# kaftanski/fissure-segmentation

Hardware: AMD Instinct MI355X
Metric: points/sec fwd+bwd DGCNN-seg N=2048 k=20 (higher is better)
Workload: dtype f32

## Files before the change

### fissure-segmentation_amd/_lib.py

```python
import ctypes
import os

import torch

_HERE = os.path.dirname(os.path.abspath(__file__))
LIB_PATH = os.environ.get("FSG_HIP_LIB") or os.path.join(_HERE, "libfsg_hip.so")

if not os.path.exists(LIB_PATH):
    raise ImportError(f"{LIB_PATH} not found: build it with `python -c 'import __graft_entry__ as g; g.build()'` "
                      f"or `make -C {os.path.join(_HERE, 'csrc')}`; there is no CPU fallback.")

lib = ctypes.CDLL(LIB_PATH)

_P, _I, _L, _F = ctypes.c_void_p, ctypes.c_int, ctypes.c_int64, ctypes.c_float
SIGNATURES = {
    "fsg_version": ([], _I),
    "fsg_last_error": ([], ctypes.c_char_p),
    "fsg_knn_dense_f32": ([_P, _I, _I, _L, _L, _I, _I, _I, _P, _P, _P, _P], _I),
    "fsg_knn_dense_workspace_bytes": ([_I, _I, _I], ctypes.c_size_t),
    "fsg_knn_dense_ws_f32": ([_P, _I, _I, _L, _L, _I, _I, _I, _P, _P, _P, ctypes.c_size_t, _P], _I),
    "fsg_knn_dense_prepared_f32": ([_P, _I, _I, _I, _I, _I, _P, _P, _P, ctypes.c_size_t, _P], _I),
    "fsg_knn_dense_ws_pq_f32": ([_P, _I, _I, _L, _L, _I, _I, _I, _P, _P, _P, ctypes.c_size_t, _P, _I, _P, _P], _I),
    "fsg_edgeconv_apply_f32": ([_P, _P, _P, _P, _P, _I, _I, _I, _F, _P, _P, _P, ctypes.c_size_t, _P], _I),
    "fsg_edgeconv_apply_pq_f32": ([_P, _P, _P, _P, _P, _I, _I, _I, _F, _P, _P, _P, ctypes.c_size_t, _P, _I, _P, _P], _I),
    "fsg_edge_gather_fwd_f32": ([_P, _P, _P, _I, _I, _I, _I, _P], _I),
    "fsg_edge_gather_bwd_f32": ([_P, _P, _P, _I, _I, _I, _I, _P], _I),
    "fsg_knn_gather_fused_f32": ([_P, _I, _I, _I, _I, _I, _P, _P, _P, _P], _I),
    "fsg_knn_gather_fused_ws_f32": ([_P, _I, _I, _I, _I, _I, _P, _P, _P, ctypes.c_size_t, _P], _I),
    "fsg_edge_gather_fwd_bf16": ([_P, _P, _P, _I, _I, _I, _I, _P], _I),
    "fsg_edge_gather_bwd_bf16": ([_P, _P, _P, _I, _I, _I, _I, _P], _I),
    "fsg_graph_reverse_csr_workspace_bytes": ([_I, _I, _I], ctypes.c_size_t),
    "fsg_graph_reverse_csr": ([_P, _I, _I, _I, _P, _P, _P, _P], _I),
    "fsg_edge_weights_fwd_f32": ([_P, _I, _I, _P, _P], _I),
    "fsg_edge_weights_bwd_f32": ([_P, _I, _I, _P, _P], _I),
    "fsg_edge_weights_many_f32": ([_P, _I, _P], _I),
    "fsg_edgeconv1_workspace_bytes": ([_I, _I, _I], ctypes.c_size_t),
    "fsg_edgeconv1_fwd_f32": ([_P, _P, _P, _P, _P, _P, _I, _I, _I, _I, _I, _F, _F, _F, _P, _P, _P, _P, _P, _P, _P, _P, _P],
                              _I),
    "fsg_edgeconv1_bwd_f32": ([_P, _P, _L, _P, _L, _P, _P, _P, _P, _P, _P, _P, _P, _P, _P, _I, _I, _I, _I, _I, _F, _P, _P,
                               _P, _P, _P, _P], _I),
    "fsg_edgeconv2_workspace_bytes": ([_I, _I, _I, _I], ctypes.c_size_t),
    "fsg_edgeconv2_bwd_workspace_bytes": ([_I, _I, _I, _I], ctypes.c_size_t),
    "fsg_edgeconv2_fwd_f32": ([_P] * 11 + [_I] * 5 + [_F] * 5 + [_P] * 12, _I),
    "fsg_edgeconv2_bwd_f32": ([_P, _P, _L, _P, _L] + [_P] * 16 + [_I] * 5 + [_F] + [_P] * 8, _I),
    "fsg_edgeconv2_fwd_bf16": ([_P] * 11 + [_I] * 5 + [_F] * 5 + [_P] * 12, _I),
    "fsg_edgeconv2_bwd_bf16": ([_P, _P, _L, _P, _L] + [_P] * 16 + [_I] * 5 + [_F] + [_P] * 8, _I),
    "fsg_bn_act_workspace_bytes": ([ctypes.c_long, _I], ctypes.c_size_t),
    "fsg_bn_act_fwd_f32": ([_P, _P, _P, _P, _P, ctypes.c_long, _I, _I, _F, _F, _F, _P, _P, _P, _P, _P], _I),
    "fsg_bn_act_bwd_f32": ([_P, _P, _P, _P, _P, _P, ctypes.c_long, _I, _I, _F, _P, _P, _P, _P, _P], _I),
    "fsg_bn_act_max_workspace_bytes": ([_I, _I, _I], ctypes.c_size_t),
    "fsg_bn_act_max_fwd_f32": ([_P, _P, _P, _P, _P, _I, _I, _I, _I, _F, _F, _F, _P, _P, _P, _P, _P, _P, _P], _I),
    "fsg_bn_act_max_bwd_f32": ([_P, _P, _P, _P, _P, _P, _P, _P, _I, _I, _I, _I, _F, _P, _P, _P, _P], _I),
    "fsg_bn_act_maxavg_workspace_bytes": ([_I, _I, _I], ctypes.c_size_t),
    "fsg_bn_act_maxavg_fwd_f32": ([_P, _P, _P, _P, _P, _I, _I, _I, _I, _F, _F, _F, _P, _P, _P, _P, _P, _P], _I),
    "fsg_bn_act_maxavg_bwd_f32": ([_P, _P, _P, _P, _P, _P, _P, _I, _I, _I, _I, _F, _P, _P, _P, _P, _P], _I),
    "fsg_chamfer_nn_f32": ([_P, _P, _I, _I, _I, _P, _P, _P], _I),
    "fsg_chamfer_nn_bwd_workspace_bytes": ([_I, _I, _I], ctypes.c_size_t),
    "fsg_chamfer_nn_bwd_f32": ([_P, _P, _P, _P, _I, _I, _I, _P, _P, _P, _P], _I),
    "fsg_point_mesh_dist_f32": ([_P, _P, _P, _I, _I, _I, _I, _I, _P, _P, _P, _P], _I),
    "fsg_mesh_labelmap_dist_f32": ([_P, _P, _P, _I, _I, _I, _I, _I, _F, _F, _F, _F, _P, _P, _P, _P], _I),
    "fsg_mesh_labelmap_cover_f32": ([_P, _P, _P, _I, _I, _I, _I, _I, _F, _F, _F, _P, _P], _I),
    "fsg_ensemble_accumulate_workspace_bytes": ([_I, _L], ctypes.c_size_t),
    "fsg_ensemble_accumulate_f32": ([_P, _I, _I, _I, _I, _P, _L, _P, _P, _P], _I),
    "fsg_sample_transform_f32": ([_P, _I, _I, _L, _P, _I, _P, _P, _P], _I),
    "fsg_ssm_decode_bwd_workspace_bytes": ([_I, _I, _I], ctypes.c_size_t),
    "fsg_ssm_decode_fwd_f32": ([_P, _P, _P, _P, _P, _P, _I, _I, _I, _P, _P], _I),
    "fsg_ssm_decode_bwd_f32": ([_P, _P, _P, _P, _P, _P, _I, _I, _I, _P, _P, _P, _P, _P, ctypes.c_size_t, _P], _I),
    "fsg_colsum_narrow_f32": ([_P, _L, _I, _P, _P], _I),
    "fsg_fold_layer1_f32": ([_P, _I, _P, _L, _P, _I, _I, _I, _I, _P, _P], _I),
    "fsg_adam_flat_f32": ([_P, _P, _P, _P, _P, _L, _F, _P, _F, _F, _F, _F, _P], _I),
    "fsg_nnu_loss_workspace_bytes": ([_I], ctypes.c_size_t),
    "fsg_nnu_loss_f32": ([_P, _L, _L, _L, _P, _P, _I, _I, _I, _F, _F, _F, _P, _P, _L, _L, _L, _P, _P], _I),
    "fsg_bn_rows_workspace_bytes": ([ctypes.c_long, _I], ctypes.c_size_t),
    "fsg_bn_rows_fwd_f32": ([_P, _P, _P, _P, _P, _P, ctypes.c_long, _I, _I, _F, _F, _I, _P, _P, _P, _P, _P], _I),
    "fsg_bn_rows_bwd_f32": ([_P, _P, _P, _P, _P, _P, ctypes.c_long, _I, _I, _I, _P, _P, _P, _P, _P, _P], _I),
    "fsg_gemm_small_workspace_bytes": ([_I, _I, _I], ctypes.c_size_t),
    "fsg_gemm_small_f32": ([_P, _L, _L, _P, _L, _L, _P, _P, _L, _I, _I, _I, _P, _P], _I),
    "fsg_gemm_small_rowsum_f32": ([_P, _L, _L, _P, _L, _L, _P, _P, _L, _I, _I, _I, _P, _P, _P], _I),
    "fsg_gemm_small_deferred_f32": ([_P, _L, _L, _P, _L, _L, _P, _L, _I, _I, _I, _P, _P, _P, _P], _I),
    "fsg_gemm_small_reduce_many_f32": ([_P, _P], _I),
    "fsg_gemm_small_bf16": ([_P, _L, _L, _P, _L, _L, _P, _P, _L, _I, _I, _I, _P, _P, _P, _P], _I),
    "fsg_pt_attn_workspace_bytes": ([_I, _I, _I], ctypes.c_size_t),
    "fsg_pt_attn_fwd_f32": ([_P, _P, _P, _P, _P, _L, _P, _I, _I, _I, _I, _P, _P, _P, _P, _P, _P], _I),
    "fsg_pt_attn_bwd_f32": ([_P, _P, _P, _P, _P, _L, _P, _I, _I, _I, _I, _P, _P, _P, _P, _P, _P, _P, _L, _P, _P, _P, _P], _I),
    "fsg_knn_segment_f32": ([_P, _P, _P, _P, _I, _I, _I, _I, _P, _P, _P], _I),
    "fsg_fps_f32": ([_P, _P, _P, _I, _I, _P, _P, _P], _I),
    "fsg_group_gather_fwd_f32": ([_P, _P, _P, _I, _I, _I, _I, _P], _I),
    "fsg_group_gather_bwd_f32": ([_P, _P, _P, _I, _I, _I, _I, _P], _I),
    "fsg_group_xyz_feat_fwd_f32": ([_P, _P, _P, _P, _P, _I, _I, _I, _I, _P], _I),
    "fsg_group_xyz_feat_bwd_f32": ([_P, _P, _P, _I, _I, _I, _I, _P], _I),
    "fsg_rows_max_fwd_f32": ([_P, _P, _P, _I, _I, _I, _P], _I),
    "fsg_rows_max_bwd_f32": ([_P, _P, _P, _I, _I, _I, _P], _I),
    "fsg_interp_fwd_f32": ([_P, _P, _P, _P, _I, _I, _I, _I, _P], _I),
    "fsg_interp_bwd_f32": ([_P, _P, _P, _P, _I, _I, _I, _I, _P], _I),
    "fsg_vec_attn_fwd_f32": ([_P, _P, _P, _P, _P, _I, _I, _I, _I, _P], _I),
    "fsg_vec_attn_bwd_f32": ([_P, _P, _P, _P, _P, _P, _P, _P, _I, _I, _I, _I, _P], _I),
    "fsg_pw_weight_image_bytes": ([_I, _I], ctypes.c_size_t),
    "fsg_pw_weight_image_f32": ([_P, _L, _L, _I, _I, _F, _I, _I, _P, _P], _I),
    "fsg_pw_weight_images_f32": ([_P, _P], _I),
    "fsg_pw_linear_f32": ([_P, _L, _P, _P, _P, _L, _I, _I, _I, _I, _P], _I),
    "fsg_pw_weight_image_bf16": ([_P, _L, _L, _I, _I, _P, _P], _I),
    "fsg_pw_linear_bf16": ([_P, _L, _P, _P, _P, _L, _I, _I, _I, _I, _P], _I),
    "fsg_pw_tn_bf16": ([_P, _I, _P, ctypes.c_size_t, _P, _L, _P], _I),
    "fsg_pw_tile_rows": ([_I], _I),
    "fsg_pw_rowgemm_f32": ([_P, _I, _I, _I, _P], _I),
    "fsg_pw_tn_workspace_bytes": ([_I, _I, _I, _I], ctypes.c_size_t),
    "fsg_pw_tn_f32": ([_P, _I, _P, ctypes.c_size_t, _P, _L, _P, _L, _P], _I),
    "fsg_pw_tn_reduce_f32": ([_P, _P], _I),
    "fsg_pw_bn_finalize_f32": ([_P, _I, _I, _I, _I, _P, _I, _I, _P, _P, _F, _F, _P, _P, _P, _P, _P, _P, _P, _P, _P, _P, _L, _I, _P, _P], _I),
    "fsg_pw_cloud_linear_f32": ([_P, _P, _L, _I, _I, _I, _P, _P], _I),
    "fsg_pw_max_finish_f32": ([_P, _P, _P, _P, _P, _I, _I, _I, _F, _P, _P, _P, _P], _I),
    "fsg_pw_bn_finalize_max_f32": ([_P, _I, _I, _I, _I, _I, _I, _P, _P, _F, _F, _P, _P, _P, _P, _P, _P, _P, _P, _P, _I, _F, _P, _P, _P,
                                   _P], _I),
    "fsg_pw_bnbwd_finalize_f32": ([_P, _I, _I, _I, _L, _I, _P, _P, _P, _I, _P, _P, _P, _P, _P, _P, _P], _I),
    "fsg_pw_logits_bwd_f32": ([_P, _I, _P, _P, _P, _P, _P, _P, _L, _I, _F, _P, _P, _P], _I),
    "fsg_pw_gf_prep_f32": ([_P, _P, _L, _I, _P, _P, _L, _P, _P, _P, _P, _P, _P, _I, _I, _L, _I, _F, _P, _P, _P, _P, _P, _P, _L, _I, _P, _L,
                            _P], _I),
    "fsg_pw_scatter_rows_workspace_bytes": ([_I, _I], ctypes.c_size_t),
    "fsg_pw_scatter_rows_f32": ([_P, _P, _P, _L, _I, _I, _I, _I, _P, _L, _P, _P], _I),
    "fsg_pw_gf_dw_f32": ([_P, _P, _P, _L, _P, _P, _L, _P, _P, _P, _I, _I, _I, _I, _P, _L, _P], _I),
    "fsg_pw_logits_bwd_bias_f32": ([_P, _I, _P, _P, _P, _P, _P, _P, _L, _I, _F, _P, _P, _P, _P], _I),
    "fsg_pw_gf_prep_sort_f32": ([_P, _P, _L, _I, _P, _P, _L, _P, _P, _P, _P, _P, _I, _I, _L, _I, _F, _P, _P, _P, _P, _P, _P, _L, _I, _P,
                                 _L, _P, _I, _P, _P, _P], _I),
    "fsg_pw_tn_reduce_image_f32": ([_P, _I, _I, _I, _I, _F, _I, _I, _P, _P, _L, _P], _I),
    "fsg_pw_rowgemm_scatter_f32": ([_P, _P, _P, _P, _P, _L, _I, _P], _I),
    "fsg_foerstner_dist_f32": ([_P, _I, _I, _I, _I, _P, _I, _P, _P], _I),
    "fsg_nms_keypoints": ([_P, _P, _I, _I, _I, _I, _I, _F, _P, _P, _P], _I),
    "fsg_mind_stats_workspace_bytes": ([_I, _I, _I, _I], ctypes.c_size_t),
    "fsg_mind_stats_f32": ([_P, _I, _I, _I, _I, _I, _I, _I, _P, _P, _I, _P, _P, _P], _I),
    "fsg_mind_eval_f32": ([_P, _I, _I, _I, _I, _I, _I, _I, _P, _P, _P, _I, _P, _P, _P], _I),
    "fsg_mind_eval_kp_f32": ([_P, _I, _I, _I, _I, _I, _I, _P, _P, _P, _I, _P, _P, _I, _P, _P], _I),
    "fsg_fissure_enhance_f32": ([_P, _P, _I, _I, _I, _I, _P, _P, _I, _F, _F, _P, _P, _P, _P], _I),
    "fsg_smooth_threshold_f32": ([_P, _I, _I, _I, _I, _P, _I, _P, _I, _P, _I, _F, _P, _P, _P], _I),
    "fsg_cpd_estep_workspace_bytes": ([_I, _I, _I], ctypes.c_size_t),
    "fsg_cpd_estep_f32": ([_P, _L, _P, _P, _F, _I, _I, _I, _P, _P, _P, _P, _P, ctypes.c_size_t, _P], _I),
    "fsg_random_walk_workspace_bytes": ([_I, _I, _I, _I, _I], ctypes.c_size_t),
    "fsg_random_walk_prep": ([_P, _I, _P, _I, _P, _I, _I, _I, _I, _I, _P, ctypes.c_size_t, _P, _P, _P], _I),
    "fsg_random_walk_iterate": ([_P, _I, _I, _I, _I, _I, _I, _I, _I, _F, _P, ctypes.c_size_t, _P, _P, _P], _I),
    "fsg_random_walk_finish": ([_I, _I, _I, _I, _I, _P, ctypes.c_size_t, _P, _P, _P], _I),
    "fsg_lobes_to_fissures_u8": ([_P, _I, _I, _I, _I, _I, _P, _P], _I),
    "fsg_bits_pack_u8": ([_P, _I, _I, _I, _I, _I, _P, _P], _I),
    "fsg_bits_unpack_u8": ([_P, _I, _I, _I, _I, _P, _P], _I),
    "fsg_bits_window": ([_P, _I, _I, _I, _I, _I, _I, _I, _I, _I, _I, _P, _P], _I),
    "fsg_ball_dilate_bits": ([_P, _I, _I, _I, _I, _I, _I, _I, _I, _I, _I, _P, _P], _I),
    "fsg_cc_workspace_bytes": ([_I, _I, _I, _I], ctypes.c_size_t),
    "fsg_cc_label_bits": ([_P, _I, _I, _I, _I, _I, _P, _P, _P, ctypes.c_size_t, _P], _I),
    "fsg_component_stats_i32": ([_P, _I, _I, _I, _I, _I, _P, _P], _I),
    "fsg_relabel_lut_i32": ([_P, _I, _L, _P, _I, _P, _I, _P], _I),
    "fsg_mesh_reg_workspace_bytes": ([_I, _I], ctypes.c_size_t),
    "fsg_mesh_reg_f32": ([_P, _L, _P, _I, _I, _P, _P, _P, _P, _P, _P, _P, _P, _P, ctypes.c_size_t, _P], _I),
    "fsg_mesh_sample_workspace_bytes": ([_I, _I], ctypes.c_size_t),
    "fsg_mesh_sample_f32": ([_P, _P, _P, _I, _I, _P, _I, _P, _P, _P, _P, ctypes.c_size_t, _P], _I),
    "fsg_mesh_sample_bwd_f32": ([_P, _P, _P, _P, _P, _I, _I, _I, _P, _P], _I),
    "fsg_grid_corners_f32": ([_P, _I, _I, _I, _I, _I, _I, _P, _P, _P], _I),
    "fsg_grid_splat_workspace_bytes": ([_I, _I, _I], ctypes.c_size_t),
    "fsg_grid_splat_sorted_f32": ([_P, _P, _P, _P, _I, _I, _I, _I, _I, _I, _P, _P, ctypes.c_size_t, _P], _I),
    "fsg_grid_sample_f32": ([_P, _P, _P, _I, _I, _I, _I, _I, _I, _I, _P, _P, _P], _I),
    "fsg_psr_spectral_f32": ([_P, _I, _I, _I, _I, ctypes.c_double, _I, _P, _P], _I),
    "fsg_mc_workspace_bytes": ([_I, _I, _I, _I], ctypes.c_size_t),
    "fsg_mc_count_f32": ([_P, _P, _L, _I, _I, _I, _I, _F, _I, _P, ctypes.c_size_t, _P, _P], _I),
    "fsg_mc_count_labels_i32": ([_P, _P, _L, _I, _I, _I, _I, _I, _P, ctypes.c_size_t, _P, _P], _I),
    "fsg_mc_emit_f32": ([_P, _I, _I, _I, _I, _F, _I, _F, _F, _F, _P, ctypes.c_size_t, _P, _L, _L, _P, _P, _P, _P], _I),
    "fsg_mc_emit_labels_i32": ([_P, _I, _I, _I, _I, _I, _I, _F, _F, _F, _P, ctypes.c_size_t, _P, _L, _L, _P, _P, _P, _P], _I),
    "fsg_pcl_normals_f32": ([_P, _P, _P, _I, _I, _I, _I, _P, _P, _P, _P], _I),
    "fsg_orient_normals_workspace_bytes": ([_I, _I], ctypes.c_size_t),
    "fsg_orient_normals_f32": ([_P, _P, _P, _P, _I, _I, _I, _P, ctypes.c_size_t, _P, _P, _P, _P], _I),
    "fsg_face_union_i32": ([_P, _P, _I, _P, _P, _P], _I),
    "fsg_cluster_stats_f64": ([_P, _P, _P, _P, _P, _I, _I, _I, _P, _P, _P, _P], _I),
    "fsg_mesh_keep_flags_u8": ([_P, _I, _P, _I, _P, _P, _P, _I, _I, _I, _F, _F, _F, _P, _P], _I),
    "fsg_mesh_face_flags_u8": ([_P, _I, _I, _P, _P, _P, _P, _P], _I),
    "fsg_mesh_compact_f32": ([_P, _P, _P, _I, _I, _P, _I, _P, _P, _P, _P, _P, _P, _P, _P], _I),
}
for _name, (_args, _res) in SIGNATURES.items():
    _fn = getattr(lib, _name)
    _fn.argtypes, _fn.restype = _args, _res

GRID_TORCH, GRID_SAP = 0, 1
MORPH_MAX_RADIUS = 8
PCL_NORMALS_MAX_K = 64
ORIENT_MAX_POINTS = 1 << 20
RW_BINARY, RW_INTENSITY, RW_MAX_LABELS = 0, 1, 8
KNN_FIX_DIAG, KNN_DROP_FIRST, KNN_FORCE_ROWS, KNN_FORCE_MFMA, KNN_MAX_K = 1, 2, 4, 8, 64
KNN_DBG_HALF_CHUNKS, KNN_DBG_TWO_PHASE, KNN_DBG_ALL_SLOW, KNN_DBG_STATS = 1 << 11, 1 << 21, 1 << 22, 1 << 25
KNN_DBG_STAMPS, KNN_DBG_ONE_LAUNCH, KNN_DBG_BF16 = 1 << 28, 1 << 29, 1 << 30


_timing = None


def start_timing():
    global _timing
    _timing = {}


def stop_timing():
    global _timing
    rec, _timing = _timing, None
    torch.cuda.synchronize()
    return {name: [s.elapsed_time(e) for s, e in evs] for name, evs in (rec or {}).items()}


class PTLayerParams(ctypes.Structure):
    _fields_ = [(n, _P) for n in ("lp1_w", "lp1_b", "bnp_g", "bnp_b", "bnp_rm", "bnp_rv", "lp2_w", "lp2_b", "bn1_g", "bn1_b",
                                  "bn1_rm", "bn1_rv", "lw1_w", "lw1_b", "bn2_g", "bn2_b", "bn2_rm", "bn2_rv", "lw2_w",
                                  "lw2_b")] + [(n, _F) for n in ("eps_p", "eps_1", "eps_2", "mom_p", "mom_1", "mom_2")]


GEMM_REDUCE_MAX_JOBS = 48


class GemmReduceJobs(ctypes.Structure):
    _fields_ = [("part", _P * GEMM_REDUCE_MAX_JOBS), ("C", _P * GEMM_REDUCE_MAX_JOBS), ("rowsum", _P * GEMM_REDUCE_MAX_JOBS),
                ("ldc", _L * GEMM_REDUCE_MAX_JOBS), ("S", _I * GEMM_REDUCE_MAX_JOBS), ("I", _I * GEMM_REDUCE_MAX_JOBS),
                ("J", _I * GEMM_REDUCE_MAX_JOBS), ("blocks", _I * GEMM_REDUCE_MAX_JOBS), ("n", _I)]


class EdgeWeightJobs(ctypes.Structure):
    _fields_ = [("src", _P * 8), ("dst", _P * 8), ("Co", _I * 8), ("C", _I * 8), ("n", _I)]


class PWRowGemmArgs(ctypes.Structure):
    _fields_ = [("A1", _P), ("Y1", _P), ("A2", _P), ("lda1", _L), ("lda2", _L), ("K1", _I), ("K2", _I), ("Bimg", _P),
                ("M", _I), ("N", _I), ("rows_per_cloud", _I), ("alpha", _P), ("delta", _P), ("P", _P), ("Q", _P),
                ("tstride", _I), ("slope", _F), ("C", _P), ("ldc", _L), ("store_n0", _I), ("bias", _P), ("rec", _P),
                ("sgn", _P), ("sel_val", _P), ("sel_arg", _P), ("sel_n", _I), ("Yp", _P), ("ldyp", _L), ("ealpha", _P),
                ("edelta", _P), ("emu", _P), ("er", _P), ("etstride", _I), ("rec2", _P)]


PW_MAX_IMAGE_JOBS = 10


class PWImageJobs(ctypes.Structure):
    _fields_ = [("W", _P * PW_MAX_IMAGE_JOBS), ("stride_n", _L * PW_MAX_IMAGE_JOBS), ("stride_k", _L * PW_MAX_IMAGE_JOBS),
                ("N", _I * PW_MAX_IMAGE_JOBS), ("K", _I * PW_MAX_IMAGE_JOBS), ("ks0", _I * PW_MAX_IMAGE_JOBS),
                ("KS", _I * PW_MAX_IMAGE_JOBS), ("scale", _F * PW_MAX_IMAGE_JOBS), ("image", _P * PW_MAX_IMAGE_JOBS), ("n", _I)]


PW_MAX_REDUCE_JOBS = 6


class PWTnReduceJobs(ctypes.Structure):
    _fields_ = [("workspace", _P * PW_MAX_REDUCE_JOBS), ("C1", _P * PW_MAX_REDUCE_JOBS), ("C2", _P * PW_MAX_REDUCE_JOBS),
                ("ldc1", _L * PW_MAX_REDUCE_JOBS), ("ldc2", _L * PW_MAX_REDUCE_JOBS), ("S", _I * PW_MAX_REDUCE_JOBS),
                ("N1", _I * PW_MAX_REDUCE_JOBS), ("N2", _I * PW_MAX_REDUCE_JOBS), ("N1a", _I * PW_MAX_REDUCE_JOBS), ("n", _I)]


class PWTnArgs(ctypes.Structure):
    _fields_ = [("L1", _P), ("LY1", _P), ("L2", _P), ("ldl1", _L), ("ldl2", _L), ("N1a", _I), ("N1b", _I), ("lpro", _I),
                ("lalpha", _P), ("ldelta", _P), ("lP", _P), ("lQ", _P), ("lts", _I), ("R", _P), ("ldr", _L), ("N2", _I),
                ("rpro", _I), ("ralpha", _P), ("rdelta", _P), ("rts", _I), ("slope", _F), ("M", _I), ("rows_per_cloud", _I),
                ("rows_per_slice", _I), ("ones", _I)]


class PTLayerGrads(ctypes.Structure):
    _fields_ = [(n, _P) for n in ("lp1_w", "lp1_b", "bnp_g", "bnp_b", "lp2_w", "lp2_b", "bn1_g", "bn1_b", "lw1_w", "lw1_b",
                                  "bn2_g", "bn2_b", "lw2_w", "lw2_b")]


_experiments = None


def experiments():
    global _experiments
    if _experiments is None:
        path = os.path.join(_HERE, "libfsg_hip_experiments.so")
        if not os.path.exists(path):
            raise ImportError(f"{path} not found: `make -C {os.path.join(_HERE, 'csrc')} all` builds it")
        x = ctypes.CDLL(path)
        x.fsg_knn_experiment_f32.argtypes, x.fsg_knn_experiment_f32.restype = SIGNATURES["fsg_knn_dense_f32"][0], _I
        x.fsg_last_error.restype = ctypes.c_char_p
        _experiments = x
    return _experiments


def workspace(entry, *dims, device):
    nbytes = getattr(lib, entry + "_workspace_bytes")(*dims)
    return torch.empty(nbytes, dtype=torch.uint8, device=device) if nbytes else None


def call(name, *args):
    if _timing is None:
        rc = getattr(lib, name)(*args)
    else:
        s, e = torch.cuda.Event(enable_timing=True), torch.cuda.Event(enable_timing=True)
        s.record()
        rc = getattr(lib, name)(*args)
        e.record()
        _timing.setdefault(name, []).append((s, e))
    if rc != 0:
        raise RuntimeError(f"{name} failed (code {rc}): {lib.fsg_last_error().decode()}")
```

### fissure-segmentation_amd/csrc/adam.hip

```cpp
#include "fsg_common.h"

namespace {

struct AdamState {
    float step;
    unsigned int ticket;
};

__device__ __forceinline__ void adam_one(float &p, float g, float &m, float &v, float b1, float b2, float eps, float wd,
                                         float step_size, float bc2_sqrt) {
    if (wd != 0.f) g = fmaf(wd, p, g);
    m = m + (1.f - b1) * (g - m);
    v = b2 * v + (1.f - b2) * g * g;
    const float denom = sqrtf(v) / bc2_sqrt + eps;
    p -= step_size * (m / denom);
}

__global__ __launch_bounds__(256) void adam_flat_kernel(float *__restrict__ param, const float *__restrict__ grad,
                                                        float *__restrict__ exp_avg, float *__restrict__ exp_avg_sq,
                                                        AdamState *__restrict__ state, long n, float lr_host,
                                                        const float *__restrict__ lr_dev, float b1, float b2, float eps,
                                                        float wd) {
    __shared__ float sc[2];
    if (threadIdx.x == 0) {
        const double t = (double)state->step + 1.0;
        const double lr = lr_dev ? (double)lr_dev[0] : (double)lr_host;
        sc[0] = (float)(lr / (1.0 - pow((double)b1, t)));
        sc[1] = (float)sqrt(1.0 - pow((double)b2, t));
    }
    __syncthreads();
    const float step_size = sc[0], bc2_sqrt = sc[1];
    const long n4 = n >> 2;
    for (long i = (long)blockIdx.x * 256 + threadIdx.x; i < n4; i += (long)gridDim.x * 256) {
        float4 p = reinterpret_cast<float4 *>(param)[i];
        const float4 g = reinterpret_cast<const float4 *>(grad)[i];
        float4 m = reinterpret_cast<float4 *>(exp_avg)[i];
        float4 v = reinterpret_cast<float4 *>(exp_avg_sq)[i];
        adam_one(p.x, g.x, m.x, v.x, b1, b2, eps, wd, step_size, bc2_sqrt);
        adam_one(p.y, g.y, m.y, v.y, b1, b2, eps, wd, step_size, bc2_sqrt);
        adam_one(p.z, g.z, m.z, v.z, b1, b2, eps, wd, step_size, bc2_sqrt);
        adam_one(p.w, g.w, m.w, v.w, b1, b2, eps, wd, step_size, bc2_sqrt);
        reinterpret_cast<float4 *>(param)[i] = p;
        reinterpret_cast<float4 *>(exp_avg)[i] = m;
        reinterpret_cast<float4 *>(exp_avg_sq)[i] = v;
    }
    if (blockIdx.x == 0 && threadIdx.x < (n & 3)) {
        const long i = (n4 << 2) + threadIdx.x;
        float p = param[i], m = exp_avg[i], v = exp_avg_sq[i];
        adam_one(p, grad[i], m, v, b1, b2, eps, wd, step_size, bc2_sqrt);
        param[i] = p;
        exp_avg[i] = m;
        exp_avg_sq[i] = v;
    }
    __syncthreads();
    if (threadIdx.x == 0) {
        const unsigned int done = atomicAdd(&state->ticket, 1u);
        if (done == gridDim.x - 1) {
            state->step += 1.f;
            state->ticket = 0u;
        }
    }
}

}

extern "C" int fsg_adam_flat_f32(float *param, const float *grad, float *exp_avg, float *exp_avg_sq, void *state, int64_t n,
                                 float lr, const float *lr_dev, float beta1, float beta2, float eps, float weight_decay,
                                 fsg_stream_t stream) {
    FSG_REQUIRE(param && grad && exp_avg && exp_avg_sq && state, "fsg_adam_flat_f32: NULL pointer");
    FSG_REQUIRE(n > 0, "fsg_adam_flat_f32: n=%ld", (long)n);
    FSG_REQUIRE((((uintptr_t)param | (uintptr_t)grad | (uintptr_t)exp_avg | (uintptr_t)exp_avg_sq) & 15) == 0,
                "fsg_adam_flat_f32: the four arrays must be 16-byte aligned");
    FSG_REQUIRE(((uintptr_t)state & 7) == 0, "fsg_adam_flat_f32: state must be 8-byte aligned");
    FSG_REQUIRE(beta1 >= 0.f && beta1 < 1.f && beta2 >= 0.f && beta2 < 1.f && eps >= 0.f,
                "fsg_adam_flat_f32: bad hyper-parameters beta1=%g beta2=%g eps=%g", beta1, beta2, eps);
    long blocks = ((n >> 2) + 255) / 256;
    if (blocks < 1) blocks = 1;
    if (blocks > 1024) blocks = 1024;
    hipLaunchKernelGGL(adam_flat_kernel, dim3((unsigned)blocks), dim3(256), 0, (hipStream_t)stream, param, grad, exp_avg,
                       exp_avg_sq, (AdamState *)state, (long)n, lr, lr_dev, beta1, beta2, eps, weight_decay);
    FSG_CHECK_LAUNCH("fsg_adam_flat_f32");
    return FSG_OK;
}
```

### fissure-segmentation_amd/csrc/small_gemm.hip

```cpp

#include "fsg_common.h"

namespace {

constexpr int TI = 64, TJ = 64, TK = 32, LDT = 65;
constexpr int LPT = TI * TK / 256;

__global__ __launch_bounds__(256) void gemm_small_kernel(const float *__restrict__ A, long sai, long sak,
                                                         const float *__restrict__ B, long sbk, long sbj,
                                                         const float *__restrict__ bias, float *__restrict__ C, long ldc,
                                                         int I, int J, int K, int kchunk, float *__restrict__ part,
                                                         float *__restrict__ rowsum) {
    __shared__ float As[TK * LDT], Bs[TK * LDT];
    const int tid = threadIdx.x, wave = __builtin_amdgcn_readfirstlane(tid >> 6), lane = tid & 63, ql = lane & 31, half = lane >> 5;
    const int i0 = blockIdx.x * TI, j0 = blockIdx.y * TJ;
    const int kbeg = blockIdx.z * kchunk, kend = min(K, kbeg + kchunk);
    const int wi = (wave >> 1) * 32, wj = (wave & 1) * 32;
    const bool a_kfast = sak == 1, b_kfast = sbk == 1;
    f32x16 acc;
#pragma unroll
    for (int e = 0; e < 16; ++e) acc[e] = 0.f;
    float av[LPT], bv[LPT];
    auto fetch = [&](int k0) {
#pragma unroll
        for (int r = 0; r < LPT; ++r) {
            const int t = r * 256 + tid;
            const int ai = a_kfast ? t / TK : t % TI, ak = a_kfast ? t % TK : t / TI;
            const int bj = b_kfast ? t / TK : t % TJ, bk = b_kfast ? t % TK : t / TJ;
            av[r] = (i0 + ai < I && k0 + ak < kend) ? A[(long)(i0 + ai) * sai + (long)(k0 + ak) * sak] : 0.f;
            bv[r] = (j0 + bj < J && k0 + bk < kend) ? B[(long)(k0 + bk) * sbk + (long)(j0 + bj) * sbj] : 0.f;
        }
    };
    const bool do_rs = rowsum != nullptr && blockIdx.y == 0 && tid < TI;
    float rs = 0.f;
    if (kbeg < kend) fetch(kbeg);
    for (int k0 = kbeg; k0 < kend; k0 += TK) {
        __syncthreads();
#pragma unroll
        for (int r = 0; r < LPT; ++r) {
            const int t = r * 256 + tid;
            const int ai = a_kfast ? t / TK : t % TI, ak = a_kfast ? t % TK : t / TI;
            const int bj = b_kfast ? t / TK : t % TJ, bk = b_kfast ? t % TK : t / TJ;
            As[ak * LDT + ai] = av[r];
            Bs[bk * LDT + bj] = bv[r];
        }
        __syncthreads();
        if (k0 + TK < kend) fetch(k0 + TK);
        if (do_rs) {
#pragma unroll
            for (int kk = 0; kk < TK; ++kk) rs += As[kk * LDT + tid];
        }
#pragma unroll
        for (int s = 0; s < TK / 2; ++s)
            acc = __builtin_amdgcn_mfma_f32_32x32x2f32(As[(2 * s + half) * LDT + wi + ql], Bs[(2 * s + half) * LDT + wj + ql],
                                                       acc, 0, 0, 0);
    }
    if (do_rs && i0 + tid < I) {
        if (part) part[(long)gridDim.z * I * J + (long)blockIdx.z * I + i0 + tid] = rs;
        else rowsum[i0 + tid] = rs;
    }
    const int col = j0 + wj + ql;
    if (col >= J) return;
    if (part) {
        float *dst = part + (long)blockIdx.z * I * J;
#pragma unroll
        for (int e = 0; e < 16; ++e) {
            const int row = i0 + wi + (e & 3) + 8 * (e >> 2) + 4 * half;
            if (row < I) dst[(long)row * J + col] = acc[e];
        }
    } else {
        const float bb = bias ? bias[col] : 0.f;
#pragma unroll
        for (int e = 0; e < 16; ++e) {
            const int row = i0 + wi + (e & 3) + 8 * (e >> 2) + 4 * half;
            if (row < I) C[(long)row * ldc + col] = acc[e] + bb;
        }
    }
}

typedef unsigned short u16;
constexpr int LDH = TK + 8;
__device__ __forceinline__ u16 to_bf16(float x) {
    const __bf16 h = (__bf16)x;
    return __builtin_bit_cast(u16, h);
}
__global__ __launch_bounds__(256) void gemm_small_bf16_kernel(const float *__restrict__ A, long sai, long sak,
                                                              const float *__restrict__ B, long sbk, long sbj,
                                                              const float *__restrict__ bias, float *__restrict__ C, long ldc,
                                                              int I, int J, int K, int kchunk, float *__restrict__ part,
                                                              float *__restrict__ rowsum) {
    __shared__ __attribute__((aligned(16))) u16 As[TI * LDH], Bs[TJ * LDH];
    const int tid = threadIdx.x, wave = __builtin_amdgcn_readfirstlane(tid >> 6), lane = tid & 63, ql = lane & 31, half = lane >> 5;
    const int i0 = blockIdx.x * TI, j0 = blockIdx.y * TJ;
    const int kbeg = blockIdx.z * kchunk, kend = min(K, kbeg + kchunk);
    const int wi = (wave >> 1) * 32, wj = (wave & 1) * 32;
    const bool a_kfast = sak == 1, b_kfast = sbk == 1;
    f32x16 acc;
#pragma unroll
    for (int e = 0; e < 16; ++e) acc[e] = 0.f;
    float av[LPT], bv[LPT];
    auto fetch = [&](int k0) {
#pragma unroll
        for (int r = 0; r < LPT; ++r) {
            const int t = r * 256 + tid;
            const int ai = a_kfast ? t / TK : t % TI, ak = a_kfast ? t % TK : t / TI;
            const int bj = b_kfast ? t / TK : t % TJ, bk = b_kfast ? t % TK : t / TJ;
            av[r] = (i0 + ai < I && k0 + ak < kend) ? A[(long)(i0 + ai) * sai + (long)(k0 + ak) * sak] : 0.f;
            bv[r] = (j0 + bj < J && k0 + bk < kend) ? B[(long)(k0 + bk) * sbk + (long)(j0 + bj) * sbj] : 0.f;
        }
    };
    const bool do_rs = rowsum != nullptr && blockIdx.y == 0 && tid < TI;
    float rs = 0.f;
    if (kbeg < kend) fetch(kbeg);
    for (int k0 = kbeg; k0 < kend; k0 += TK) {
        __syncthreads();
#pragma unroll
        for (int r = 0; r < LPT; ++r) {
            const int t = r * 256 + tid;
            const int ai = a_kfast ? t / TK : t % TI, ak = a_kfast ? t % TK : t / TI;
            const int bj = b_kfast ? t / TK : t % TJ, bk = b_kfast ? t % TK : t / TJ;
            As[ai * LDH + ak] = to_bf16(av[r]);
            Bs[bj * LDH + bk] = to_bf16(bv[r]);
        }
        __syncthreads();
        if (k0 + TK < kend) fetch(k0 + TK);
        if (do_rs) {
#pragma unroll
            for (int kk = 0; kk < TK; ++kk) rs += __uint_as_float((unsigned)As[tid * LDH + kk] << 16);
        }
#pragma unroll
        for (int s = 0; s < TK / 16; ++s) {
            const bf16x8 a = *reinterpret_cast<const bf16x8 *>(&As[(wi + ql) * LDH + 16 * s + 8 * half]);
            const bf16x8 b = *reinterpret_cast<const bf16x8 *>(&Bs[(wj + ql) * LDH + 16 * s + 8 * half]);
            acc = __builtin_amdgcn_mfma_f32_32x32x16_bf16(a, b, acc, 0, 0, 0);
        }
    }
    if (do_rs && i0 + tid < I) {
        if (part) part[(long)gridDim.z * I * J + (long)blockIdx.z * I + i0 + tid] = rs;
        else rowsum[i0 + tid] = rs;
    }
    const int col = j0 + wj + ql;
    if (col >= J) return;
    if (part) {
        float *dst = part + (long)blockIdx.z * I * J;
#pragma unroll
        for (int e = 0; e < 16; ++e) {
            const int row = i0 + wi + (e & 3) + 8 * (e >> 2) + 4 * half;
            if (row < I) dst[(long)row * J + col] = acc[e];
        }
    } else {
        const float bb = bias ? bias[col] : 0.f;
#pragma unroll
        for (int e = 0; e < 16; ++e) {
            const int row = i0 + wi + (e & 3) + 8 * (e >> 2) + 4 * half;
            if (row < I) C[(long)row * ldc + col] = acc[e] + bb;
        }
    }
}

__global__ __launch_bounds__(256) void gemm_small_reduce_flat_kernel(const float *__restrict__ part, int S, long IJ, int J,
                                                                     const float *__restrict__ bias, float *__restrict__ C,
                                                                     long ldc, int I, float *__restrict__ rowsum) {
    const long t = (long)blockIdx.x * 256 + threadIdx.x;
    if (rowsum && t >= IJ && t < IJ + I) {
        float a = 0.f;
        for (int s = 0; s < S; ++s) a += part[(long)S * IJ + (long)s * I + (t - IJ)];
        rowsum[t - IJ] = a;
    }
    if (t >= IJ) return;
    float a = 0.f;
    for (int s = 0; s < S; ++s) a += part[(long)s * IJ + t];
    const long row = t / J;
    const int col = (int)(t - row * J);
    C[row * ldc + col] = a + (bias ? bias[col] : 0.f);
}

__global__ __launch_bounds__(256) void gemm_small_reduce_kernel(const float *__restrict__ part, int S, long IJ, int J,
                                                                const float *__restrict__ bias, float *__restrict__ C,
                                                                long ldc, int I, float *__restrict__ rowsum) {
    __shared__ float red[16][17];
    const int o = threadIdx.x & 15, sl = threadIdx.x >> 4;
    const long t = (long)blockIdx.x * 16 + o;
    const long nb = (IJ + 15) / 16;
    if (rowsum && (long)blockIdx.x >= nb) {
        const long ri = ((long)blockIdx.x - nb) * 16 + o;
        float a = 0.f;
        if (ri < I)
            for (int s = sl; s < S; s += 16) a += part[(long)S * IJ + (long)s * I + ri];
        red[sl][o] = a;
        __syncthreads();
        if (sl == 0 && ri < I) {
            float r = 0.f;
#pragma unroll
            for (int i = 0; i < 16; ++i) r += red[i][o];
            rowsum[ri] = r;
        }
        return;
    }
    float a = 0.f;
    if (t < IJ)
        for (int s = sl; s < S; s += 16) a += part[(long)s * IJ + t];
    red[sl][o] = a;
    __syncthreads();
    if (sl == 0 && t < IJ) {
        float r = 0.f;
#pragma unroll
        for (int i = 0; i < 16; ++i) r += red[i][o];
        const long row = t / J;
        const int col = (int)(t - row * J);
        C[row * ldc + col] = r + (bias ? bias[col] : 0.f);
    }
}

__global__ __launch_bounds__(256) void gemm_small_reduce_many_kernel(fsg_gemm_reduce_jobs jobs) {
    int j = 0;
    long b = blockIdx.x;
    while (j < jobs.n - 1 && b >= jobs.blocks[j]) { b -= jobs.blocks[j]; ++j; }
    const float *part = jobs.part[j];
    const int S = jobs.S[j], I = jobs.I[j], J = jobs.J[j];
    const long IJ = (long)I * J, t = b * 256 + threadIdx.x;
    float *rowsum = jobs.rowsum[j];
    if (rowsum && t >= IJ && t < IJ + I) {
        float a = 0.f;
        for (int s = 0; s < S; ++s) a += part[(long)S * IJ + (long)s * I + (t - IJ)];
        rowsum[t - IJ] = a;
    }
    if (t >= IJ) return;
    float a = 0.f;
#pragma unroll 8
    for (int s = 0; s < S; ++s) a += part[(long)s * IJ + t];
    const long row = t / J;
    const int col = (int)(t - row * J);
    jobs.C[j][row * jobs.ldc[j] + col] = a;
}

inline int splits_for(int I, int J, int K) {
    constexpr int min_k = 64;
    const long tiles = (long)fsg_cdiv(I, TI) * fsg_cdiv(J, TJ);
    if (tiles >= 256 || K < 2 * min_k) return 1;
    long s = (1024 + tiles - 1) / tiles;
    const long smax = K / min_k;
    if (s > smax) s = smax;
    if (s > 128) s = 128;
    return s < 1 ? 1 : (int)s;
}

}

extern "C" size_t fsg_gemm_small_workspace_bytes(int I, int J, int K) {
    if (I <= 0 || J <= 0 || K <= 0) return 0;
    const int s = splits_for(I, J, K);
    return s > 1 ? sizeof(float) * (size_t)s * ((size_t)I * (size_t)J + (size_t)I) : 0;
}

extern "C" int fsg_gemm_small_rowsum_f32(const float *A, int64_t sa_i, int64_t sa_k, const float *B, int64_t sb_k, int64_t sb_j,
                                         const float *bias, float *C, int64_t ldc, int I, int J, int K, float *rowsum,
                                         void *workspace, fsg_stream_t stream);

extern "C" int fsg_gemm_small_f32(const float *A, int64_t sa_i, int64_t sa_k, const float *B, int64_t sb_k, int64_t sb_j,
                                  const float *bias, float *C, int64_t ldc, int I, int J, int K, void *workspace,
                                  fsg_stream_t stream) {
    return fsg_gemm_small_rowsum_f32(A, sa_i, sa_k, B, sb_k, sb_j, bias, C, ldc, I, J, K, nullptr, workspace, stream);
}

namespace {
int gemm_small_launch(const float *A, int64_t sa_i, int64_t sa_k, const float *B, int64_t sb_k, int64_t sb_j, const float *bias,
                      float *C, int64_t ldc, int I, int J, int K, float *rowsum, void *workspace, int *deferred_splits,
                      fsg_stream_t stream, bool bf16 = false);
}

extern "C" int fsg_gemm_small_rowsum_f32(const float *A, int64_t sa_i, int64_t sa_k, const float *B, int64_t sb_k, int64_t sb_j,
                                         const float *bias, float *C, int64_t ldc, int I, int J, int K, float *rowsum,
                                         void *workspace, fsg_stream_t stream) {
    return gemm_small_launch(A, sa_i, sa_k, B, sb_k, sb_j, bias, C, ldc, I, J, K, rowsum, workspace, nullptr, stream);
}

extern "C" int fsg_gemm_small_deferred_f32(const float *A, int64_t sa_i, int64_t sa_k, const float *B, int64_t sb_k, int64_t sb_j,
                                           float *C, int64_t ldc, int I, int J, int K, float *rowsum, void *workspace, int *splits,
                                           fsg_stream_t stream) {
    FSG_REQUIRE(splits, "fsg_gemm_small_deferred_f32: NULL splits");
    return gemm_small_launch(A, sa_i, sa_k, B, sb_k, sb_j, nullptr, C, ldc, I, J, K, rowsum, workspace, splits, stream);
}

extern "C" int fsg_gemm_small_bf16(const float *A, int64_t sa_i, int64_t sa_k, const float *B, int64_t sb_k, int64_t sb_j,
                                   const float *bias, float *C, int64_t ldc, int I, int J, int K, float *rowsum, void *workspace,
                                   int *splits, fsg_stream_t stream) {
    FSG_REQUIRE(!(splits && bias), "fsg_gemm_small_bf16: a deferred product takes no bias");
    return gemm_small_launch(A, sa_i, sa_k, B, sb_k, sb_j, bias, C, ldc, I, J, K, rowsum, workspace, splits, stream, true);
}

extern "C" int fsg_gemm_small_reduce_many_f32(const fsg_gemm_reduce_jobs *jobs, fsg_stream_t stream) {
    FSG_REQUIRE(jobs && jobs->n >= 1 && jobs->n <= FSG_GEMM_REDUCE_MAX_JOBS, "fsg_gemm_small_reduce_many_f32: bad job count");
    fsg_gemm_reduce_jobs j = *jobs;
    long total = 0;
    for (int i = 0; i < j.n; ++i) {
        FSG_REQUIRE(j.part[i] && j.C[i] && j.S[i] >= 1 && j.I[i] > 0 && j.J[i] > 0 && j.ldc[i] >= j.J[i],
                    "fsg_gemm_small_reduce_many_f32: bad job %d", i);
        j.blocks[i] = (int)fsg_cdiv((long)j.I[i] * j.J[i] + (j.rowsum[i] ? j.I[i] : 0), 256L);
        total += j.blocks[i];
    }
    FSG_REQUIRE(total < (1L << 31), "fsg_gemm_small_reduce_many_f32: too many outputs");
    hipLaunchKernelGGL(gemm_small_reduce_many_kernel, dim3((unsigned)total), dim3(256), 0, (hipStream_t)stream, j);
    FSG_CHECK_LAUNCH("fsg_gemm_small_reduce_many_f32");
    return FSG_OK;
}

namespace {
int gemm_small_launch(const float *A, int64_t sa_i, int64_t sa_k, const float *B, int64_t sb_k, int64_t sb_j, const float *bias,
                      float *C, int64_t ldc, int I, int J, int K, float *rowsum, void *workspace, int *deferred_splits,
                      fsg_stream_t stream, bool bf16) {
    FSG_REQUIRE(A && B && C, "fsg_gemm_small_f32: NULL pointer");
    FSG_REQUIRE(I > 0 && J > 0 && K > 0 && ldc >= J, "fsg_gemm_small_f32: bad shape I=%d J=%d K=%d ldc=%ld", I, J, K, (long)ldc);
    FSG_REQUIRE(fsg_cdiv(J, TJ) <= 65535, "fsg_gemm_small_f32: J too large");
    const int S = splits_for(I, J, K);
    FSG_REQUIRE(S == 1 || workspace, "fsg_gemm_small_f32: this shape needs the workspace");
    hipStream_t st = (hipStream_t)stream;
    int kchunk = fsg_cdiv(fsg_cdiv(K, S), TK) * TK;
    const int S_eff = fsg_cdiv(K, kchunk);
    float *part = S_eff > 1 ? (float *)workspace : nullptr;
    if (bf16)
        hipLaunchKernelGGL(gemm_small_bf16_kernel, dim3(fsg_cdiv(I, TI), fsg_cdiv(J, TJ), S_eff), dim3(256), 0, st, A, (long)sa_i,
                           (long)sa_k, B, (long)sb_k, (long)sb_j, bias, C, (long)ldc, I, J, K, kchunk, part, rowsum);
    else
        hipLaunchKernelGGL(gemm_small_kernel, dim3(fsg_cdiv(I, TI), fsg_cdiv(J, TJ), S_eff), dim3(256), 0, st, A, (long)sa_i,
                           (long)sa_k, B, (long)sb_k, (long)sb_j, bias, C, (long)ldc, I, J, K, kchunk, part, rowsum);
    FSG_CHECK_LAUNCH("fsg_gemm_small_f32");
    if (deferred_splits) {
        *deferred_splits = part ? S_eff : 0;
        return FSG_OK;
    }
    if (part) {
        const long IJ = (long)I * J, outs = IJ + (rowsum ? I : 0);
        if (S_eff >= 16)
            hipLaunchKernelGGL(gemm_small_reduce_kernel, dim3(fsg_cdiv(IJ, 16) + (rowsum ? fsg_cdiv(I, 16) : 0)), dim3(256), 0, st, part,
                               S_eff, IJ, J, bias, C, (long)ldc, I, rowsum);
        else
            hipLaunchKernelGGL(gemm_small_reduce_flat_kernel, dim3(fsg_cdiv(outs, 256)), dim3(256), 0, st, part, S_eff, IJ, J,
                               bias, C, (long)ldc, I, rowsum);
        FSG_CHECK_LAUNCH("fsg_gemm_small_f32/reduce");
    }
    return FSG_OK;
}
}
```

### fissure-segmentation_amd/functional.py

```python
import contextlib as _contextlib
import ctypes
import os as _os

import torch

from . import _lib


def _need_gpu(*tensors):
    for t in tensors:
        if t is not None and not t.is_cuda:
            raise RuntimeError("fissure_segmentation_amd runs on the GPU only (got a CPU tensor); "
                               "the CPU restatement lives in oracle/ and is test infrastructure")


def _p(t):
    return ctypes.c_void_p(t.data_ptr() if t is not None else 0)


def _stream():
    return ctypes.c_void_p(torch.cuda.current_stream().cuda_stream)


def _f32c(t):
    return t.detach().to(torch.float32).contiguous()


def _amp_fwd(fn):
    return torch.amp.custom_fwd(fn, device_type="cuda", cast_inputs=torch.float32)


def _amp_bwd(fn):
    return torch.amp.custom_bwd(fn, device_type="cuda")


def no_autocast():
    if torch.is_autocast_enabled("cuda"):
        return torch.autocast("cuda", enabled=False)
    return _contextlib.nullcontext()


_mfma_mode = "f32"


def set_mfma_operands(kind):
    global _mfma_mode
    if kind not in ("f32", "bf16"):
        raise ValueError("MFMA operand type must be 'f32' or 'bf16'")
    _mfma_mode = kind


@_contextlib.contextmanager
def mfma_operands(kind):
    global _mfma_mode
    old = _mfma_mode
    set_mfma_operands(kind)
    try:
        yield
    finally:
        _mfma_mode = old


def bf16_operands():
    return _mfma_mode == "bf16"


def _ambient_bf16():
    return torch.is_autocast_enabled("cuda") and torch.get_autocast_dtype("cuda") == torch.bfloat16


_deterministic = bool(_os.environ.get("FSG_DETERMINISTIC"))


def set_deterministic(flag=True):
    global _deterministic
    _deterministic = bool(flag)


def deterministic():
    return _deterministic or torch.are_deterministic_algorithms_enabled()


def knn_graph(x, k, c_knn=None, fix_diag=True, drop_first=False, return_dist=False, force_rows_kernel=False,
              _debug_flags=0, out=None, prepared=None, pq_weight=None):
    _need_gpu(x)
    if x.dim() != 3:
        raise ValueError(f"expected (B,C,N), got {tuple(x.shape)}")
    x = x.detach()
    if x.dtype != torch.float32:
        x = x.float()
    if x.stride(2) != 1:
        x = x.contiguous()
    B, C, N = x.shape
    c_knn = C if c_knn is None else c_knn
    if out is not None:
        if out.shape != (B, N, k) or out.dtype != torch.int32 or not out.is_contiguous() or out.device != x.device:
            raise ValueError("knn_graph: `out` must be a contiguous (B,N,k) int32 tensor on the input's device")
        idx = out
    else:
        idx = torch.empty(B, N, k, dtype=torch.int32, device=x.device)
    dist = torch.empty(B, N, k, dtype=torch.float32, device=x.device) if return_dist else None
    flags = (_lib.KNN_FIX_DIAG if fix_diag else 0) | (_lib.KNN_DROP_FIRST if drop_first else 0) | \
        (_lib.KNN_FORCE_ROWS if force_rows_kernel else 0) | _debug_flags
    if prepared is not None and c_knn == C and not return_dist and not force_rows_kernel and not _debug_flags:
        ws, x_pm = prepared
        with torch.cuda.device(x.device):
            _lib.call("fsg_knn_dense_prepared_f32", _p(x_pm), B, N, C, k, flags, _p(idx), None, _p(ws), ws.numel() * ws.element_size(),
                      _stream())
        return idx
    xx = _lib.workspace("fsg_knn_dense", B, N, c_knn, device=x.device)
    ws_bytes = xx.numel() if xx is not None else 0
    if pq_weight is not None:
        rows = pq_weight.shape[0]
        if (C == c_knn and c_knn <= 4 and tuple(pq_weight.shape) == (rows, C) and 256 % rows == 0 and not return_dist and
                not (_debug_flags & _lib.KNN_FORCE_MFMA)):
            pq = torch.empty(B, N, rows, dtype=torch.float32, device=x.device)
            with torch.cuda.device(x.device):
                _lib.call("fsg_knn_dense_ws_pq_f32", _p(x), B, N, x.stride(0), x.stride(1), c_knn, k, flags, _p(idx), None, _p(xx),
                          ws_bytes, _p(_f32c(pq_weight.detach())), rows, _p(pq), _stream())
            return idx, pq
    with torch.cuda.device(x.device):
        rc = 3
        if flags & _lib.KNN_FORCE_MFMA:
            xl = _lib.experiments()
            rc = xl.fsg_knn_experiment_f32(_p(x), B, N, x.stride(0), x.stride(1), c_knn, k, flags, _p(idx), _p(dist), _p(xx),
                                           _stream())
            if rc not in (0, 3):
                raise RuntimeError(xl.fsg_last_error().decode())
        if rc == 3:
            _lib.call("fsg_knn_dense_ws_f32", _p(x), B, N, x.stride(0), x.stride(1), c_knn, k, flags & ~_lib.KNN_FORCE_MFMA, _p(idx),
                      _p(dist), _p(xx), ws_bytes, _stream())
    if pq_weight is not None:
        return idx, None
    return (idx, dist) if return_dist else idx


class _EdgeGather(torch.autograd.Function):
    @staticmethod
    @_amp_fwd
    def forward(ctx, x, idx):
        B, C, N = x.shape
        k = idx.shape[2]
        half = x.dtype == torch.bfloat16
        xc = x.detach().contiguous() if half else _f32c(x)
        out = torch.empty(B, 2 * C, N, k, dtype=xc.dtype, device=x.device)
        with torch.cuda.device(x.device):
            _lib.call("fsg_edge_gather_fwd_bf16" if half else "fsg_edge_gather_fwd_f32", _p(xc), _p(idx), _p(out), B, C, N, k,
                      _stream())
        ctx.save_for_backward(idx)
        ctx.shape = (B, C, N, k)
        ctx.half = half
        return out

    @staticmethod
    @_amp_bwd
    def backward(ctx, g):
        (idx,) = ctx.saved_tensors
        B, C, N, k = ctx.shape
        half = ctx.half and g.dtype == torch.bfloat16
        g = g.detach().contiguous() if half else _f32c(g)
        gx = torch.empty(B, C, N, dtype=torch.float32, device=g.device)
        with torch.cuda.device(g.device):
            _lib.call("fsg_edge_gather_bwd_bf16" if half else "fsg_edge_gather_bwd_f32", _p(g), _p(idx), _p(gx), B, C, N, k,
                      _stream())
        return (gx.to(torch.bfloat16) if ctx.half else gx), None


def knn_edge_features(x, k, knn_only_over_coords=False):
    _need_gpu(x)
    xc = _f32c(x)
    B, C, N = xc.shape
    idx = torch.empty(B, N, k, dtype=torch.int32, device=x.device)
    edge = torch.empty(B, 2 * C, N, k, dtype=torch.float32, device=x.device)
    c_knn = 3 if knn_only_over_coords else C
    ws = _lib.workspace("fsg_knn_dense", B, N, c_knn, device=x.device)
    with torch.cuda.device(x.device):
        _lib.call("fsg_knn_gather_fused_ws_f32", _p(xc), B, C, N, k, c_knn, _p(idx), _p(edge), _p(ws), ws.numel(), _stream())
    return edge, idx


def edge_features(x, idx):
    _need_gpu(x, idx)
    if idx.dtype != torch.int32:
        idx = idx.to(torch.int32)
    return _EdgeGather.apply(x, idx.contiguous())


SMALL_GEMM_FLOPS = 6e8


def gemm_small(a, sa_i, sa_k, b, sb_k, sb_j, bias, I, J, K, rowsum=False, defer=False, bf16=False):
    out = torch.empty(I, J, dtype=torch.float32, device=a.device)
    ws = _lib.workspace("fsg_gemm_small", I, J, K, device=a.device)
    rs = torch.empty(I, dtype=torch.float32, device=a.device) if rowsum else None
    with torch.cuda.device(a.device):
        if defer and bias is None:
            splits = ctypes.c_int(0)
            if bf16:
                _lib.call("fsg_gemm_small_bf16", _p(a), sa_i, sa_k, _p(b), sb_k, sb_j, None, _p(out), J, I, J, K, _p(rs), _p(ws),
                          ctypes.byref(splits), _stream())
            else:
                _lib.call("fsg_gemm_small_deferred_f32", _p(a), sa_i, sa_k, _p(b), sb_k, sb_j, _p(out), J, I, J, K, _p(rs), _p(ws),
                          ctypes.byref(splits), _stream())
            if splits.value > 1:
                _defer_reduce((ws, out.data_ptr(), rs.data_ptr() if rs is not None else None, splits.value, I, J, a.device))
        elif bf16:
            _lib.call("fsg_gemm_small_bf16", _p(a), sa_i, sa_k, _p(b), sb_k, sb_j, _p(bias), _p(out), J, I, J, K, _p(rs), _p(ws), None,
                      _stream())
        else:
            _lib.call("fsg_gemm_small_rowsum_f32", _p(a), sa_i, sa_k, _p(b), sb_k, sb_j, _p(bias), _p(out), J, I, J, K, _p(rs),
                      _p(ws), _stream())
    return (out, rs) if rowsum else out


_pending_reduces = []
_defer_weight_grads = True


def set_deferred_weight_grads(flag):
    global _defer_weight_grads
    _defer_weight_grads = bool(flag)


def _grad_targets(w):
    if w.is_leaf:
        return (w,)
    return getattr(w, "_fsg_grad_unread", None)


def _may_defer(targets):
    return (_defer_weight_grads and targets is not None and not torch.is_grad_enabled() and
            all(p.grad is None for p in targets))


def flush_deferred_reduces():
    global _pending_reduces
    jobs, _pending_reduces = _pending_reduces, []
    for i0 in range(0, len(jobs), _lib.GEMM_REDUCE_MAX_JOBS):
        chunk = jobs[i0:i0 + _lib.GEMM_REDUCE_MAX_JOBS]
        tab = _lib.GemmReduceJobs()
        for i, (ws, out, rs, S, I, J, _dev) in enumerate(chunk):
            tab.part[i], tab.C[i], tab.rowsum[i] = ws.data_ptr(), out, rs
            tab.ldc[i], tab.S[i], tab.I[i], tab.J[i] = J, S, I, J
        tab.n = len(chunk)
        with torch.cuda.device(chunk[0][6]):
            _lib.call("fsg_gemm_small_reduce_many_f32", ctypes.byref(tab), _stream())


def _defer_reduce(job):
    _pending_reduces.append(job)
    try:
        torch.autograd.Variable._execution_engine.queue_callback(flush_deferred_reduces)
    except RuntimeError:
        flush_deferred_reduces()


def _small(I, J, K, *tensors):
    if not all(t.is_cuda and t.dtype == torch.float32 and t.is_contiguous() for t in tensors):
        return False
    vol = float(I) * J * K
    return 0 < I <= 256 and 0 < J <= 256 and (1 << 21) <= vol and 2.0 * vol < SMALL_GEMM_FLOPS


class _LinearPM(torch.autograd.Function):

    @staticmethod
    @_amp_fwd
    def forward(ctx, x, w, b):
        ctx.save_for_backward(x, w)
        ctx.has_bias = b is not None
        ctx.pw16 = False
        tw, tb = _grad_targets(w), (_grad_targets(b) if b is not None else ())
        ctx.defer_targets = tw + tb if (tw is not None and tb is not None) else None
        x2 = x.reshape(-1, x.shape[-1])
        N, K = w.shape
        M = x2.shape[0]
        ctx.gs16 = (_bf16_linear and bf16_operands() and M > 0 and
                    all(t.is_cuda and t.dtype == torch.float32 and t.is_contiguous() for t in (x2, w)))
        if ctx.gs16:
            y = gemm_small(x2, K, 1, w, 1, K, b.contiguous() if b is not None else None, M, N, K, bf16=True)
            return y if x.dim() == 2 else y.view(*x.shape[:-1], N)
        if not (_bf16_linear and bf16_operands()) and _small(M, N, K, x2, w):
            y = gemm_small(x2, K, 1, w, 1, K, b.contiguous() if b is not None else None, M, N, K)
            return y if x.dim() == 2 else y.view(*x.shape[:-1], N)
        ctx.pw16 = _pw_bf16_ok(x2, w)
        if ctx.pw16:
            y = torch.empty(*x.shape[:-1], N, dtype=torch.float32, device=x.device)
            pw_linear_bf16(x2, w, b, out=y.view(-1, N))
            return y
        return torch.nn.functional.linear(x, w, b)

    @staticmethod
    @_amp_bwd
    def backward(ctx, g):
        x, w = ctx.saved_tensors
        g2 = g.reshape(-1, g.shape[-1])
        x2 = x.reshape(-1, x.shape[-1])
        gx = gw = gb = None
        if not g2.is_contiguous():
            g2 = g2.contiguous()
        if ctx.gs16:
            N, K = w.shape
            M = g2.shape[0]
            if ctx.needs_input_grad[0]:
                gx = gemm_small(g2, N, 1, w, K, 1, None, M, K, N, bf16=True).view_as(x)
            want_gb = ctx.has_bias and ctx.needs_input_grad[2]
            if ctx.needs_input_grad[1]:
                x2c = x2 if x2.is_contiguous() else x2.contiguous()
                gw = gemm_small(g2, 1, N, x2c, K, 1, None, N, K, M, rowsum=want_gb, defer=_may_defer(ctx.defer_targets), bf16=True)
                if want_gb:
                    gw, gb = gw
            elif want_gb:
                gb = _bias_grad(g2)
            return gx, gw, gb
        if ctx.pw16:
            if ctx.needs_input_grad[0]:
                gx = (pw_linear_bf16(g2, w.t(), None) if w.shape[0] % 32 == 0 else g2 @ w).view_as(x)
            if ctx.needs_input_grad[1]:
                gw = pw_tn_bf16(g2, x2 if x2.is_contiguous() else x2.contiguous())
            if ctx.has_bias and ctx.needs_input_grad[2]:
                gb = _bias_grad(g2)
            return gx, gw, gb
        if ctx.needs_input_grad[0]:
            gx = _linear_dx(g2, w).view_as(x)
        want_gb = ctx.has_bias and ctx.needs_input_grad[2]
        if ctx.needs_input_grad[1]:
            gw = _linear_dw(g2, x2, with_bias_grad=want_gb, defer=_may_defer(ctx.defer_targets))
            if isinstance(gw, tuple):
                gw, gb = gw
        if want_gb and gb is None:
            gb = _bias_grad(g2)
        return gx, gw, gb


def _linear_dx(g2, w, out=None):
    N, K = w.shape
    M = g2.shape[0]
    if out is not None:
        return out.addmm_(g2, w)
    return gemm_small(g2, N, 1, w, K, 1, None, M, K, N) if _small(M, K, N, g2, w) else g2 @ w


def _linear_dw(g2, x2, with_bias_grad=False, defer=False):
    M, N = g2.shape
    K = x2.shape[1]
    S = 16 if (M % 16 == 0 and M >= 4096) else 1
    if _small(N, K, M, g2, x2):
        return gemm_small(g2, 1, N, x2, K, 1, None, N, K, M, rowsum=with_bias_grad, defer=defer)
    if S > 1 and x2.is_contiguous():
        return torch.bmm(g2.view(S, M // S, -1).transpose(1, 2), x2.view(S, M // S, -1)).sum(0)
    return g2.t() @ x2


def _bias_grad(g2):
    M, N = g2.shape
    if g2.is_cuda and g2.dtype == torch.float32 and N <= 32 and (N & (N - 1)) == 0 and 4096 <= M * N <= 131072:
        out = torch.empty(N, dtype=torch.float32, device=g2.device)
        with torch.cuda.device(g2.device):
            _lib.call("fsg_colsum_narrow_f32", _p(g2), M, N, _p(out), _stream())
        return out
    return g2.sum(0)


class _LinearPMGiven(torch.autograd.Function):

    @staticmethod
    @_amp_fwd
    def forward(ctx, x, w, value):
        ctx.save_for_backward(x, w)
        return value.view_as(value)

    @staticmethod
    @_amp_bwd
    def backward(ctx, g):
        x, w = ctx.saved_tensors
        g2 = g.reshape(-1, g.shape[-1])
        if not g2.is_contiguous():
            g2 = g2.contiguous()
        x2 = x.reshape(-1, x.shape[-1])
        gx = _linear_dx(g2, w).view_as(x) if ctx.needs_input_grad[0] else None
        gw = _linear_dw(g2, x2 if x2.is_contiguous() else x2.contiguous()) if ctx.needs_input_grad[1] else None
        return gx, gw, None


def linear_pm(x, w, b=None):
    return _LinearPM.apply(x, w, b)


class _LinearPM2(torch.autograd.Function):

    @staticmethod
    @_amp_fwd
    def forward(ctx, x, w1, w2):
        ctx.save_for_backward(x, w1, w2)
        x2 = x.reshape(-1, x.shape[-1])
        return torch.nn.functional.linear(x2, w1), torch.nn.functional.linear(x2, w2)

    @staticmethod
    @_amp_bwd
    def backward(ctx, g1, g2):
        x, w1, w2 = ctx.saved_tensors
        x2 = x.reshape(-1, x.shape[-1])
        gs = [g.contiguous() if g is not None else None for g in (g1, g2)]
        gx = None
        if ctx.needs_input_grad[0]:
            for g, w in zip(gs, (w1, w2)):
                if g is not None:
                    gx = _linear_dx(g, w) if gx is None else _linear_dx(g, w, out=gx)
            gx = gx.view_as(x) if gx is not None else None
        gw1 = _linear_dw(gs[0], x2) if (gs[0] is not None and ctx.needs_input_grad[1]) else None
        gw2 = _linear_dw(gs[1], x2) if (gs[1] is not None and ctx.needs_input_grad[2]) else None
        return gx, gw1, gw2


def linear_pm2(x, w1, w2):
    return _LinearPM2.apply(x, w1, w2)


class _SplitCols(torch.autograd.Function):

    @staticmethod
    @_amp_fwd
    def forward(ctx, w, c0):
        ctx.c0, ctx.c1 = c0, w.shape[1] - c0
        return w[:, :c0], w[:, c0:]

    @staticmethod
    @_amp_bwd
    def backward(ctx, ga, gb):
        if ga is None or gb is None:
            ref = ga if ga is not None else gb
            ga = ga if ga is not None else torch.zeros(ref.shape[0], ctx.c0, dtype=ref.dtype, device=ref.device)
            gb = gb if gb is not None else torch.zeros(ref.shape[0], ctx.c1, dtype=ref.dtype, device=ref.device)
        return torch.cat([ga, gb], dim=1), None


def split_cols(w, c0):
    return _SplitCols.apply(w, c0)


_ones_memo = {}


def _ones(*shape_and_device):
    *shape, device = shape_and_device
    key = (tuple(shape), str(device))
    t = _ones_memo.get(key)
    if t is None:
        if len(_ones_memo) > 64:
            _ones_memo.clear()
        t = _ones_memo[key] = torch.ones(*shape, dtype=torch.float32, device=device)
    return t


class _AddPerCloud(torch.autograd.Function):

    @staticmethod
    @_amp_fwd
    def forward(ctx, y, c):
        return y + c.unsqueeze(1)

    @staticmethod
    @_amp_bwd
    def backward(ctx, g):
        B, N, C = g.shape
        gc = g if g.is_contiguous() else g.contiguous()
        return g, torch.bmm(_ones(B, 1, N, g.device), gc).view(B, C)


def add_per_cloud(y, c):
    return _AddPerCloud.apply(y, c)


class _LinearReLU(torch.autograd.Function):

    @staticmethod
    @_amp_fwd
    def forward(ctx, x, w, b):
        x2 = x.reshape(-1, x.shape[-1])
        out = torch._addmm_activation(b, x2, w.t(), use_gelu=False)
        ctx.save_for_backward(x, w, out)
        return out.view(*x.shape[:-1], w.shape[0])

    @staticmethod
    @_amp_bwd
    def backward(ctx, g):
        x, w, out = ctx.saved_tensors
        g2 = torch.ops.aten.threshold_backward(g.reshape(-1, g.shape[-1]).contiguous(), out, 0)
        x2 = x.reshape(-1, x.shape[-1])
        gx = _linear_dx(g2, w).view_as(x) if ctx.needs_input_grad[0] else None
        gw = _linear_dw(g2, x2) if ctx.needs_input_grad[1] else None
        gb = _bias_grad(g2) if ctx.needs_input_grad[2] else None
        return gx, gw, gb


def linear_pm_relu(x, w, b):
    _need_gpu(x, w, b)
    return _LinearReLU.apply(x, w, b)


class _FoldLayer1(torch.autograd.Function):

    @staticmethod
    @_amp_fwd
    def forward(ctx, pts, w_p, per_cloud, relu):
        pts, per_cloud = _f32c(pts), _f32c(per_cloud)
        B, m, cp = pts.shape
        Cout = w_p.shape[0]
        if w_p.dtype != torch.float32 or w_p.stride(1) != 1:
            w_p = w_p.float().contiguous()
        out = torch.empty(B, m, Cout, dtype=torch.float32, device=pts.device)
        with torch.cuda.device(pts.device):
            _lib.call("fsg_fold_layer1_f32", _p(pts), cp, _p(w_p), w_p.stride(0), _p(per_cloud), B, m, Cout, int(relu), _p(out),
                      _stream())
        ctx.save_for_backward(pts, w_p, out)
        ctx.relu = bool(relu)
        return out

    @staticmethod
    @_amp_bwd
    def backward(ctx, g):
        pts, w_p, out = ctx.saved_tensors
        B, m, cp = pts.shape
        Cout = w_p.shape[0]
        g = g.contiguous()
        if ctx.relu:
            g = torch.ops.aten.threshold_backward(g, out, 0)
        g2 = g.view(B * m, Cout)
        g_pts = (g2 @ w_p).view(B, m, cp) if ctx.needs_input_grad[0] else None
        g_w = _linear_dw(g2, pts.view(B * m, cp)) if ctx.needs_input_grad[1] else None
        g_pc = torch.bmm(_ones(B, 1, m, g.device), g).view(B, Cout) if ctx.needs_input_grad[2] else None
        return g_pts, g_w, g_pc, None


def fold_layer1(pts, w_p, per_cloud, relu=True):
    _need_gpu(pts, w_p, per_cloud)
    return _FoldLayer1.apply(pts, w_p, per_cloud, relu)


class _EdgeWeights(torch.autograd.Function):

    @staticmethod
    @_amp_fwd
    def forward(ctx, W):
        Co, C2 = W.shape
        Wc = W if (W.dtype == torch.float32 and W.is_contiguous()) else W.float().contiguous()
        out = torch.empty(2 * Co, C2 // 2, dtype=torch.float32, device=W.device)
        with torch.cuda.device(W.device):
            _lib.call("fsg_edge_weights_fwd_f32", _p(Wc), Co, C2 // 2, _p(out), _stream())
        return out

    @staticmethod
    @_amp_bwd
    def backward(ctx, g):
        Co, C = g.shape[0] // 2, g.shape[1]
        gc = g if (g.dtype == torch.float32 and g.is_contiguous()) else g.float().contiguous()
        out = torch.empty(Co, 2 * C, dtype=torch.float32, device=g.device)
        with torch.cuda.device(g.device):
            _lib.call("fsg_edge_weights_bwd_f32", _p(gc), Co, C, _p(out), _stream())
        return out


class _EdgeWeightsMany(torch.autograd.Function):

    @staticmethod
    def _run(srcs, shapes, backward):
        dev = srcs[0].device
        jobs = _lib.EdgeWeightJobs()
        jobs.n = len(srcs)
        outs = []
        for j, (t, (Co, C)) in enumerate(zip(srcs, shapes)):
            out = torch.empty((Co, 2 * C) if backward else (2 * Co, C), dtype=torch.float32, device=dev)
            jobs.src[j], jobs.dst[j], jobs.Co[j], jobs.C[j] = t.data_ptr(), out.data_ptr(), Co, C
            outs.append(out)
        with torch.cuda.device(dev):
            _lib.call("fsg_edge_weights_many_f32", ctypes.byref(jobs), int(backward), _stream())
        return outs

    @staticmethod
    @_amp_fwd
    def forward(ctx, *Ws):
        Wc = [W if (W.dtype == torch.float32 and W.is_contiguous()) else W.float().contiguous() for W in Ws]
        ctx.shapes = [(W.shape[0], W.shape[1] // 2) for W in Wc]
        return tuple(_EdgeWeightsMany._run(Wc, ctx.shapes, False))

    @staticmethod
    @_amp_bwd
    def backward(ctx, *gs):
        dev = next(g for g in gs if g is not None).device
        gc = [torch.zeros(2 * Co, C, dtype=torch.float32, device=dev) if g is None else
              (g if (g.dtype == torch.float32 and g.is_contiguous()) else g.float().contiguous())
              for g, (Co, C) in zip(gs, ctx.shapes)]
        return tuple(_EdgeWeightsMany._run(gc, ctx.shapes, True))


def edge_weights_many(conv_weights):
    Ws = [w.reshape(w.shape[0], w.shape[1]) for w in conv_weights]
    if not 1 <= len(Ws) <= 8:
        raise ValueError("edge_weights_many: 1..8 layers")
    return list(_EdgeWeightsMany.apply(*Ws))


_deferred_counters = None


def bump_bn_counter(bn):
    if bn.momentum is None:
        bn.num_batches_tracked.add_(1)
        return 1.0 / float(bn.num_batches_tracked)
    if _deferred_counters is not None:
        _deferred_counters.append(bn.num_batches_tracked)
    else:
        bn.num_batches_tracked.add_(1)
    return bn.momentum


@_contextlib.contextmanager
def deferred_bn_counters():
    global _deferred_counters
    if _deferred_counters is not None:
        yield
        return
    _deferred_counters = []
    try:
        yield
    finally:
        pending, _deferred_counters = _deferred_counters, None
        if pending:
            torch._foreach_add_(pending, 1)


def with_deferred_bn_counters(forward):
    import functools

    @functools.wraps(forward)
    def wrapped(self, x, *args, **kwargs):
        mode = mfma_operands("bf16") if (x.is_cuda and _ambient_bf16()) else _contextlib.nullcontext()
        with deferred_bn_counters(), mode, no_autocast():
            if torch.is_tensor(x) and x.is_floating_point() and x.dtype != torch.float32:
                x = x.float()
            return forward(self, x, *args, **kwargs)
    return wrapped


def _bn_step(bn):
    training = bn.training or bn.running_mean is None
    momentum = 0.0
    if training and bn.track_running_stats and bn.num_batches_tracked is not None:
        momentum = bump_bn_counter(bn)
    return training, float(momentum)


def _bn_args(bn):
    if bn.weight is None or bn.bias is None:
        raise ValueError("the fused BatchNorm stages need weight and bias: got a BatchNorm with affine=False")
    training, momentum = _bn_step(bn)
    stats = bn.track_running_stats or not training
    return (bn.weight, bn.bias, bn.running_mean if stats else None, bn.running_var if stats else None, training, momentum,
            float(bn.eps))


def _bn_eval_stats(rm, rv, eps):
    return rm.detach().float().contiguous(), torch.rsqrt(rv.detach().float() + eps).contiguous()


def _build_csr(idx):
    B, N, k = idx.shape
    rowptr = torch.empty(B, N + 1, dtype=torch.int32, device=idx.device)
    col = torch.empty(B, N * k, dtype=torch.int32, device=idx.device)
    ws = _lib.workspace("fsg_graph_reverse_csr", B, N, k, device=idx.device)
    with torch.cuda.device(idx.device):
        _lib.call("fsg_graph_reverse_csr", _p(idx), B, N, k, _p(rowptr), _p(col), _p(ws), _stream())
    return rowptr, col


def knn_prep_workspace(B, N, C, device):
    if C != 64 or N % 64 != 0 or not (1024 <= N <= 8192):
        return None
    return _lib.workspace("fsg_knn_dense", B, N, C, device=device)


def build_reverse_graphs(graphs):
    g0 = graphs[0]
    G = len(graphs)
    B, N, k = g0.shape
    step = B * N * k * g0.element_size()
    if any(g.shape != g0.shape or g.data_ptr() != g0.data_ptr() + i * step or not g.is_contiguous() for i, g in enumerate(graphs)):
        return
    if all(getattr(g, "_fsg_csr", None) is not None for g in graphs):
        return
    flat = torch.as_strided(g0, (G * B, N, k), (N * k, k, 1))
    rowptr, col = _build_csr(flat)
    for i, g in enumerate(graphs):
        g._fsg_csr = (rowptr[i * B:(i + 1) * B], col[i * B:(i + 1) * B])


def reverse_graph(idx):
    cached = getattr(idx, "_fsg_csr", None)
    if cached is None:
        cached = idx._fsg_csr = _build_csr(idx)
    return cached


def _pm_grad(g, B, N, C):
    if g is None:
        return None, 0
    if g.dtype == torch.float32 and g.shape == (B, N, C) and g.stride(2) == 1 and g.stride(1) >= C and \
            (B == 1 or g.stride(0) == N * g.stride(1)):
        return g, g.stride(1)
    return _f32c(g), C


def _apply_pass(ysel, gamma, beta, mean, invstd, B, N, Co, slope, out, out_pm, knn_ws, w_next):
    if knn_ws is None:
        return None
    nb = knn_ws.numel() * knn_ws.element_size()
    if w_next is not None and Co == 64 and tuple(w_next.shape) == (128, 64):
        w_next = _f32c(w_next.detach())
        pq_next = torch.empty(B, N, 128, dtype=torch.float32, device=ysel.device)
        _lib.call("fsg_edgeconv_apply_pq_f32", _p(ysel), _p(gamma), _p(beta), _p(mean), _p(invstd), B, N, Co, slope, _p(out),
                  _p(out_pm), _p(knn_ws), nb, _p(w_next), 128, _p(pq_next), _stream())
        return pq_next
    _lib.call("fsg_edgeconv_apply_f32", _p(ysel), _p(gamma), _p(beta), _p(mean), _p(invstd), B, N, Co, slope, _p(out),
              _p(out_pm), _p(knn_ws), nb, _stream())
    return None


class _EdgeConv1(torch.autograd.Function):
    @staticmethod
    @_amp_fwd
    def forward(ctx, pq, idx, gamma, beta, running_mean, running_var, training, momentum, eps, slope, knn_ws=None, w_next=None):
        pq = _f32c(pq)
        B, N, two_co = pq.shape
        Co, k, dev = two_co // 2, idx.shape[2], pq.device
        gamma, beta = _f32c(gamma), _f32c(beta)
        out = torch.empty(B, Co, N, dtype=torch.float32, device=dev)
        out_pm = torch.empty(B, N, Co, dtype=torch.float32, device=dev)
        ysel = torch.empty(B, N, Co, dtype=torch.float32, device=dev)
        arg = torch.empty(B, N, Co, dtype=torch.uint8, device=dev)
        if training:
            ssum = torch.empty(B, N, Co, dtype=torch.float32, device=dev)
            mean = torch.empty(Co, dtype=torch.float32, device=dev)
            invstd = torch.empty(Co, dtype=torch.float32, device=dev)
            ws = _lib.workspace("fsg_edgeconv1", B, N, Co, device=dev)
        else:
            ssum, ws = None, None
            mean, invstd = _bn_eval_stats(running_mean, running_var, eps)
        with torch.cuda.device(dev):
            _lib.call("fsg_edgeconv1_fwd_f32", _p(pq), _p(idx), _p(gamma), _p(beta),
                      _p(running_mean if training else None), _p(running_var if training else None), B, N, k, Co,
                      int(training), momentum, eps, slope, _p(None if knn_ws is not None else out), _p(out_pm), _p(ysel), _p(arg),
                      _p(ssum), _p(mean), _p(invstd), _p(ws), _stream())
            pq_next = _apply_pass(ysel, gamma, beta, mean, invstd, B, N, Co, slope, out, out_pm, knn_ws, w_next)
        ctx.save_for_backward(pq, idx, gamma, beta, mean, invstd, ysel, arg, ssum)
        ctx.meta = (B, N, k, Co, bool(training), slope)
        ctx.set_materialize_grads(False)
        if pq_next is None:
            return out, out_pm, out_pm.view(B, N, Co)
        ctx.mark_non_differentiable(pq_next)
        return out, out_pm, out_pm.view(B, N, Co), pq_next

    @staticmethod
    @_amp_bwd
    def backward(ctx, g, g_pm, g_pm2, _g_pq_next=None):
        pq, idx, gamma, beta, mean, invstd, ysel, arg, ssum = ctx.saved_tensors
        B, N, k, Co, training, slope = ctx.meta
        dev = pq.device
        g = _f32c(g) if g is not None else None
        g_pm, ld1 = _pm_grad(g_pm, B, N, Co)
        g_pm2, ld2 = _pm_grad(g_pm2, B, N, Co)
        rowptr, col = reverse_graph(idx)
        gpq = torch.empty_like(pq)
        dgamma = torch.empty(Co, dtype=torch.float32, device=dev)
        dbeta = torch.empty(Co, dtype=torch.float32, device=dev)
        h = torch.empty(B, N, Co, dtype=torch.float32, device=dev)
        ws = torch.empty(B * ((N + 63) // 64) * 2 * Co, dtype=torch.float32, device=dev)
        with torch.cuda.device(dev):
            _lib.call("fsg_edgeconv1_bwd_f32", _p(g), _p(g_pm), ld1, _p(g_pm2), ld2, _p(pq), _p(rowptr), _p(col), _p(gamma),
                      _p(beta), _p(mean),
                      _p(invstd), _p(ysel), _p(arg), _p(ssum), B, N, k, Co, int(training), slope, _p(gpq), _p(dgamma),
                      _p(dbeta), _p(h), _p(ws), _stream())
        return gpq, None, dgamma, dbeta, None, None, None, None, None, None, None, None


def edgeconv1_supported(out_channels, k):
    return out_channels % 64 == 0 and k <= 64


def edgeconv1(x, idx, conv_weight, bn, slope, x_pm=None, both=False, w_cat=None, knn_ws=None, w_next=None, pq_given=None):
    _need_gpu(x, idx, conv_weight)
    Co, C2 = conv_weight.shape[0], conv_weight.shape[1]
    C = C2 // 2
    if w_cat is None:
        w_cat = _EdgeWeights.apply(conv_weight.reshape(Co, C2).to(torch.float32))
    if x_pm is None:
        x_pm = x.transpose(1, 2)
    if pq_given is not None:
        pq = _LinearPMGiven.apply(x_pm.to(torch.float32), w_cat, pq_given)
    else:
        pq = linear_pm(x_pm.to(torch.float32).contiguous(), w_cat)
    bn_args = _bn_args(bn)
    if idx.dtype != torch.int32:
        idx = idx.to(torch.int32)
    idx = idx.contiguous()
    res = _EdgeConv1.apply(pq, idx, *bn_args, float(slope), knn_ws, w_next if knn_ws is not None else None)
    return _edgeconv_outputs(res, both, w_next is not None)


class _EdgeConv2(torch.autograd.Function):
    @staticmethod
    @_amp_fwd
    def forward(ctx, pq, idx, w2, g1, b1, rm1, rv1, g2, b2, rm2, rv2, training, mom1, mom2, eps1, eps2, slope, knn_ws=None,
                w_next=None):
        pq, w2 = _f32c(pq), _f32c(w2)
        g1, b1, g2, b2 = _f32c(g1), _f32c(b1), _f32c(g2), _f32c(b2)
        B, N, _ = pq.shape
        C2, k, dev = w2.shape[0], idx.shape[2], pq.device

        def new(*shape, dtype=torch.float32):
            return torch.empty(*shape, dtype=dtype, device=dev)
        out, out_pm = new(B, C2, N), new(B, N, C2)
        ysel2, arg2 = new(B, N, C2), new(B, N, C2, dtype=torch.uint8)
        if training:
            ssum1, ssum2 = new(B, N, 64), new(B, N, C2)
            mean1, invstd1, mean2, invstd2 = new(64), new(64), new(C2), new(C2)
        else:
            ssum1 = ssum2 = None
            mean1, invstd1 = _bn_eval_stats(rm1, rv1, eps1)
            mean2, invstd2 = _bn_eval_stats(rm2, rv2, eps2)
        ws = _lib.workspace("fsg_edgeconv2", B, N, k, C2, device=dev)
        t = bool(training)
        ctx.bf16 = bf16_operands()
        with torch.cuda.device(dev):
            _lib.call("fsg_edgeconv2_fwd_bf16" if ctx.bf16 else "fsg_edgeconv2_fwd_f32", _p(pq), _p(idx), _p(w2), _p(g1), _p(b1),
                      _p(rm1 if t else None),
                      _p(rv1 if t else None), _p(g2), _p(b2), _p(rm2 if t else None), _p(rv2 if t else None), B, N, k, C2,
                      int(t), mom1, mom2, eps1, eps2, slope, _p(None if knn_ws is not None else out), _p(out_pm), _p(ssum1), _p(mean1),
                      _p(invstd1), _p(ysel2), _p(arg2), _p(ssum2), _p(mean2), _p(invstd2), _p(ws), _stream())
            pq_next = _apply_pass(ysel2, g2, b2, mean2, invstd2, B, N, C2, slope, out, out_pm, knn_ws, w_next)
        ctx.save_for_backward(pq, idx, w2, g1, b1, mean1, invstd1, ssum1, g2, b2, mean2, invstd2, ysel2, arg2)
        ctx.meta = (B, N, k, C2, t, slope)
        ctx.set_materialize_grads(False)
        if pq_next is None:
            return out, out_pm, out_pm.view(B, N, C2)
        ctx.mark_non_differentiable(pq_next)
        return out, out_pm, out_pm.view(B, N, C2), pq_next

    @staticmethod
    @_amp_bwd
    def backward(ctx, g, g_pm, g_pm2, _g_pq_next=None):
        pq, idx, w2, g1, b1, mean1, invstd1, ssum1, g2, b2, mean2, invstd2, ysel2, arg2 = ctx.saved_tensors
        B, N, k, C2, training, slope = ctx.meta
        dev = pq.device
        g = _f32c(g) if g is not None else None
        g_pm, ld1 = _pm_grad(g_pm, B, N, C2)
        g_pm2, ld2 = _pm_grad(g_pm2, B, N, C2)
        rowptr, col = reverse_graph(idx)
        gpq, gw2 = torch.empty_like(pq), torch.empty_like(w2)
        dg1, db1 = torch.empty_like(g1), torch.empty_like(b1)
        dg2, db2 = torch.empty_like(g2), torch.empty_like(b2)
        ws = _lib.workspace("fsg_edgeconv2_bwd", B, N, k, C2, device=dev)
        with torch.cuda.device(dev):
            _lib.call("fsg_edgeconv2_bwd_bf16" if ctx.bf16 else "fsg_edgeconv2_bwd_f32", _p(g), _p(g_pm), ld1, _p(g_pm2), ld2,
                      _p(pq), _p(idx), _p(rowptr), _p(col),
                      _p(w2), _p(g1),
                      _p(b1), _p(mean1), _p(invstd1), _p(ssum1), _p(g2), _p(b2), _p(mean2), _p(invstd2), _p(ysel2),
                      _p(arg2), B, N, k, C2, int(training), slope, _p(gpq), _p(gw2), _p(dg1), _p(db1), _p(dg2), _p(db2),
                      _p(ws), _stream())
        return (gpq, None, gw2, dg1, db1, None, None, dg2, db2) + (None,) * 10


def edgeconv2_supported(c_mid, c_out, k):
    return c_mid == 64 and c_out in (64, 128) and k <= 64


def _edgeconv_outputs(res, both, want_pq_next):
    out, out_pm, out_pm2 = res[:3]
    pq_next = res[3] if len(res) > 3 else None
    if both == "twice":
        r = (out, out_pm, out_pm2)
    elif both:
        r = (out, out_pm)
    else:
        r = (out,)
    if want_pq_next:
        return r + (pq_next,)
    return r if len(r) > 1 else r[0]


def edgeconv2(x, idx, conv1_weight, bn1, conv2_weight, bn2, slope, x_pm=None, both=False, w_cat=None, knn_ws=None, w_next=None,
              pq_given=None):
    _need_gpu(x, idx, conv1_weight, conv2_weight)
    C1, CC = conv1_weight.shape[0], conv1_weight.shape[1]
    C = CC // 2
    if w_cat is None:
        w_cat = _EdgeWeights.apply(conv1_weight.reshape(C1, CC).to(torch.float32))
    if x_pm is None:
        x_pm = x.transpose(1, 2)
    if pq_given is not None:
        pq = _LinearPMGiven.apply(x_pm.to(torch.float32), w_cat, pq_given)
    else:
        pq = linear_pm(x_pm.to(torch.float32).contiguous(), w_cat)
    w2 = conv2_weight.reshape(conv2_weight.shape[0], C1)
# ... 2352 lines not shown
```

### fissure-segmentation_amd/optim.py

```python
import ctypes

import torch


class FlatAdam:
    def __init__(self, params, lr=1e-3, betas=(0.9, 0.999), eps=1e-8, weight_decay=0.0, capturable=False):
        self.params = [p for p in params if p.requires_grad]
        if not self.params:
            raise ValueError("no trainable parameters")
        dev = self.params[0].device
        if any(p.device != dev or p.dtype != torch.float32 for p in self.params):
            raise ValueError("FlatAdam needs fp32 parameters on one device")
        sizes = [p.numel() for p in self.params]
        flat = torch.empty(sum(sizes), dtype=torch.float32, device=dev)
        off = 0
        with torch.no_grad():
            for p, n in zip(self.params, sizes):
                flat[off:off + n].copy_(p.reshape(-1))
                p.data = flat[off:off + n].view(p.shape)
                off += n
        self.flat = torch.nn.Parameter(flat)
        self.flat.grad = torch.zeros_like(flat)
        self._views, self._spans = [], []
        off = 0
        for n in sizes:
            self._views.append(self.flat.grad[off:off + n])
            self._spans.append((off, off + n))
            off += n
        self.inner = None
        if dev.type == "cuda":
            self._groups = [dict(params=self.params, lr=lr, betas=tuple(betas), eps=eps, weight_decay=weight_decay)]
            self.exp_avg, self.exp_avg_sq = torch.zeros_like(flat), torch.zeros_like(flat)
            self._state = torch.zeros(2, dtype=torch.float32, device=dev)
        else:
            self.inner = torch.optim.Adam([self.flat], lr=lr, betas=betas, eps=eps, weight_decay=weight_decay)

    @property
    def param_groups(self):
        return self.inner.param_groups if self.inner is not None else self._groups

    def zero_grad(self, set_to_none=True):
        for p in self.params:
            if set_to_none:
                p.grad = None
            elif p.grad is not None:
                p.grad.zero_()

    def gather_grads(self):
        if self.flat.is_cuda:
            from . import functional as F_hip
            F_hip.flush_deferred_reduces()
        grads = [p.grad.reshape(-1) if p.grad is not None else torch.zeros_like(v) for p, v in zip(self.params, self._views)]
        torch.cat(grads, out=self.flat.grad)
        return self.flat.grad

    def step_flat(self):
        if self.inner is not None:
            self.inner.step()
            return
        from . import _lib
        g = self._groups[0]
        lr = g["lr"]
        lr_dev = None
        if isinstance(lr, torch.Tensor):
            if lr.device != self.flat.device or lr.dtype != torch.float32 or lr.numel() != 1:
                raise ValueError("a tensor learning rate must be one fp32 element on the parameters' device")
            lr_dev, lr = ctypes.c_void_p(lr.data_ptr()), 0.0
        P = lambda t: ctypes.c_void_p(t.data_ptr())
        _lib.call("fsg_adam_flat_f32", P(self.flat.data), P(self.flat.grad), P(self.exp_avg), P(self.exp_avg_sq),
                  P(self._state), self.flat.numel(), float(lr), lr_dev, float(g["betas"][0]), float(g["betas"][1]),
                  float(g["eps"]), float(g["weight_decay"]), ctypes.c_void_p(torch.cuda.current_stream().cuda_stream))

    def step(self):
        missing = [i for i, p in enumerate(self.params) if p.grad is None]
        self.gather_grads()
        if not missing or self.inner is not None:
            self.step_flat()
            return
        keep = [(a, b, self.flat.data[a:b].clone(), self.exp_avg[a:b].clone(), self.exp_avg_sq[a:b].clone())
                for a, b in (self._spans[i] for i in missing)]
        self.step_flat()
        with torch.no_grad():
            for a, b, w, m, v in keep:
                self.flat.data[a:b].copy_(w)
                self.exp_avg[a:b].copy_(m)
                self.exp_avg_sq[a:b].copy_(v)

    def state_dict(self):
        if self.inner is not None:
            return self.inner.state_dict()
        group = {k: v for k, v in self._groups[0].items() if k != "params"}
        group.update(amsgrad=False, maximize=False, foreach=None, capturable=False, differentiable=False, fused=None,
                     decoupled_weight_decay=False)
        if isinstance(group["lr"], torch.Tensor):
            group["lr"] = float(group["lr"])
        group["params"] = list(range(len(self.params)))
        step = self._state[0].detach().cpu().clone()
        state = {}
        if float(step) > 0:
            for i, (p, (a, b)) in enumerate(zip(self.params, self._spans)):
                state[i] = {"step": step.clone(), "exp_avg": self.exp_avg[a:b].view(p.shape).clone(),
                            "exp_avg_sq": self.exp_avg_sq[a:b].view(p.shape).clone()}
        return {"state": state, "param_groups": [group]}

    def load_state_dict(self, sd):
        if self.inner is not None:
            self.inner.load_state_dict(sd)
            return
        st = sd["state"]
        with torch.no_grad():
            self._state.zero_(), self.exp_avg.zero_(), self.exp_avg_sq.zero_()
            if len(st) == 1 and 0 in st and st[0]["exp_avg"].numel() == self.flat.numel() and len(self.params) > 1:
                self._state[0] = float(st[0]["step"])
                self.exp_avg.copy_(st[0]["exp_avg"].reshape(-1))
                self.exp_avg_sq.copy_(st[0]["exp_avg_sq"].reshape(-1))
            elif st:
                steps = {float(v["step"]) for v in st.values()}
                if len(steps) != 1:
                    raise ValueError("FlatAdam keeps one step counter; the checkpoint has per-parameter steps " + str(steps))
                self._state[0] = steps.pop()
                for i, v in st.items():
                    a, b = self._spans[int(i)]
                    if v["exp_avg"].numel() != b - a:
                        raise ValueError(f"optimizer state {i} does not match parameter {i}")
                    self.exp_avg[a:b].copy_(v["exp_avg"].reshape(-1))
                    self.exp_avg_sq[a:b].copy_(v["exp_avg_sq"].reshape(-1))
        for k, v in sd["param_groups"][0].items():
            if k != "params" and k in self._groups[0]:
                self._groups[0][k] = tuple(v) if k == "betas" else v
```

### include/fsg_hip.h

```cpp
#ifndef FSG_HIP_H
#define FSG_HIP_H

#include <stddef.h>
#include <stdint.h>

#ifdef __cplusplus
extern "C" {
#endif

#define FSG_OK 0
#define FSG_ERR_ARG 1
#define FSG_ERR_HIP 2
#define FSG_ERR_UNSUPPORTED 3

#define FSG_KNN_FIX_DIAG 1
#define FSG_KNN_DROP_FIRST 2

#define FSG_KNN_FORCE_ROWS 4

#define FSG_KNN_FORCE_MFMA 8

#define FSG_KNN_MAX_K 64

typedef void *fsg_stream_t;

int fsg_version(void);
const char *fsg_last_error(void);

int fsg_knn_dense_f32(const float *x, int B, int N, int64_t stride_b, int64_t stride_c, int c_knn,
                      int k, int flags, int32_t *idx_out, float *dist_out, float *xx_scratch,
                      fsg_stream_t stream);

size_t fsg_knn_dense_workspace_bytes(int B, int N, int c_knn);
int fsg_knn_dense_ws_f32(const float *x, int B, int N, int64_t stride_b, int64_t stride_c, int c_knn,
                         int k, int flags, int32_t *idx_out, float *dist_out, void *workspace,
                         size_t workspace_bytes, fsg_stream_t stream);

int fsg_knn_dense_ws_pq_f32(const float *x, int B, int N, int64_t stride_b, int64_t stride_c, int c_knn, int k, int flags,
                            int32_t *idx_out, float *dist_out, void *workspace, size_t workspace_bytes, const float *w_pq,
                            int rows_pq, float *pq_out, fsg_stream_t stream);

int fsg_knn_dense_prepared_f32(const float *x_pm, int B, int N, int c_knn, int k, int flags, int32_t *idx_out, float *dist_out,
                               void *workspace, size_t workspace_bytes, fsg_stream_t stream);

int fsg_edge_gather_fwd_f32(const float *x, const int32_t *idx, float *edge, int B, int C, int N,
                            int k, fsg_stream_t stream);
int fsg_edge_gather_bwd_f32(const float *grad_edge, const int32_t *idx, float *grad_x, int B, int C,
                            int N, int k, fsg_stream_t stream);
int fsg_knn_gather_fused_f32(const float *x, int B, int C, int N, int k, int c_knn, int32_t *idx_out, float *edge,
                             float *xx_scratch, fsg_stream_t stream);
int fsg_knn_gather_fused_ws_f32(const float *x, int B, int C, int N, int k, int c_knn, int32_t *idx_out, float *edge,
                                void *workspace, size_t workspace_bytes, fsg_stream_t stream);
int fsg_edge_gather_fwd_bf16(const void *x, const int32_t *idx, void *edge, int B, int C, int N, int k,
                             fsg_stream_t stream);
int fsg_edge_gather_bwd_bf16(const void *grad_edge, const int32_t *idx, float *grad_x, int B, int C, int N,
                             int k, fsg_stream_t stream);

size_t fsg_graph_reverse_csr_workspace_bytes(int B, int N, int k);
int fsg_graph_reverse_csr(const int32_t *idx, int B, int N, int k, int32_t *rowptr, int32_t *col,
                          void *workspace, fsg_stream_t stream);

int fsg_edge_weights_fwd_f32(const float *W, int Co, int C, float *Wt, fsg_stream_t stream);
int fsg_edge_weights_bwd_f32(const float *grad_Wt, int Co, int C, float *grad_W, fsg_stream_t stream);
#define FSG_EDGE_WEIGHT_MAX_JOBS 8
typedef struct fsg_edge_weight_jobs {
    const float *src[FSG_EDGE_WEIGHT_MAX_JOBS];
    float *dst[FSG_EDGE_WEIGHT_MAX_JOBS];
    int Co[FSG_EDGE_WEIGHT_MAX_JOBS];
    int C[FSG_EDGE_WEIGHT_MAX_JOBS];
    int n;
} fsg_edge_weight_jobs;
int fsg_edge_weights_many_f32(const fsg_edge_weight_jobs *jobs, int backward, fsg_stream_t stream);

int fsg_edgeconv_apply_f32(const float *ysel, const float *gamma, const float *beta, const float *mean, const float *invstd,
                           int B, int N, int Co, float slope, float *out, float *out_pm, void *knn_workspace,
                           size_t knn_workspace_bytes, fsg_stream_t stream);

int fsg_edgeconv_apply_pq_f32(const float *ysel, const float *gamma, const float *beta, const float *mean, const float *invstd,
                              int B, int N, int Co, float slope, float *out, float *out_pm, void *knn_workspace,
                              size_t knn_workspace_bytes, const float *w_next, int rows_next, float *pq_next,
                              fsg_stream_t stream);

size_t fsg_edgeconv1_workspace_bytes(int B, int N, int Co);
int fsg_edgeconv1_fwd_f32(const float *pq, const int32_t *idx, const float *gamma, const float *beta,
                          float *running_mean, float *running_var, int B, int N, int k, int Co, int training,
                          float momentum, float eps, float slope, float *out, float *out_pm, float *ysel,
                          uint8_t *arg, float *ssum, float *mean, float *invstd, float *workspace,
                          fsg_stream_t stream);
int fsg_edgeconv1_bwd_f32(const float *grad_out, const float *grad_out_pm, int64_t ld_pm, const float *grad_out_pm2,
                          int64_t ld_pm2, const float *pq, const int32_t *rowptr, const int32_t *col,
                          const float *gamma, const float *beta, const float *mean, const float *invstd,
                          const float *ysel, const uint8_t *arg, const float *ssum, int B, int N, int k, int Co,
                          int training, float slope, float *grad_pq, float *grad_gamma, float *grad_beta,
                          float *h_scratch, float *workspace, fsg_stream_t stream);

size_t fsg_edgeconv2_workspace_bytes(int B, int N, int k, int C2);
size_t fsg_edgeconv2_bwd_workspace_bytes(int B, int N, int k, int C2);
int fsg_edgeconv2_fwd_f32(const float *pq, const int32_t *idx, const float *w2, const float *gamma1,
                          const float *beta1, float *running_mean1, float *running_var1, const float *gamma2,
                          const float *beta2, float *running_mean2, float *running_var2, int B, int N, int k, int C2,
                          int training, float momentum1, float momentum2, float eps1, float eps2, float slope,
                          float *out, float *out_pm, float *ssum1, float *mean1, float *invstd1, float *ysel2,
                          uint8_t *arg2, float *ssum2, float *mean2, float *invstd2, void *workspace,
                          fsg_stream_t stream);
int fsg_edgeconv2_bwd_f32(const float *grad_out, const float *grad_out_pm, int64_t ld_pm, const float *grad_out_pm2,
                          int64_t ld_pm2, const float *pq, const int32_t *idx,
                          const int32_t *rowptr, const int32_t *col, const float *w2, const float *gamma1,
                          const float *beta1, const float *mean1, const float *invstd1, const float *ssum1,
                          const float *gamma2, const float *beta2, const float *mean2, const float *invstd2,
                          const float *ysel2, const uint8_t *arg2, int B, int N, int k, int C2, int training,
                          float slope, float *grad_pq, float *grad_w2, float *grad_gamma1, float *grad_beta1,
                          float *grad_gamma2, float *grad_beta2, void *workspace, fsg_stream_t stream);
int fsg_edgeconv2_fwd_bf16(const float *pq, const int32_t *idx, const float *w2, const float *gamma1,
                           const float *beta1, float *running_mean1, float *running_var1, const float *gamma2,
                           const float *beta2, float *running_mean2, float *running_var2, int B, int N, int k, int C2,
                           int training, float momentum1, float momentum2, float eps1, float eps2, float slope,
                           float *out, float *out_pm, float *ssum1, float *mean1, float *invstd1, float *ysel2,
                           uint8_t *arg2, float *ssum2, float *mean2, float *invstd2, void *workspace,
                           fsg_stream_t stream);
int fsg_edgeconv2_bwd_bf16(const float *grad_out, const float *grad_out_pm, int64_t ld_pm, const float *grad_out_pm2,
                           int64_t ld_pm2, const float *pq, const int32_t *idx,
                           const int32_t *rowptr, const int32_t *col, const float *w2, const float *gamma1,
                           const float *beta1, const float *mean1, const float *invstd1, const float *ssum1,
                           const float *gamma2, const float *beta2, const float *mean2, const float *invstd2,
                           const float *ysel2, const uint8_t *arg2, int B, int N, int k, int C2, int training,
                           float slope, float *grad_pq, float *grad_w2, float *grad_gamma1, float *grad_beta1,
                           float *grad_gamma2, float *grad_beta2, void *workspace, fsg_stream_t stream);

size_t fsg_bn_act_workspace_bytes(long M, int C);
int fsg_bn_act_fwd_f32(const float *y, const float *gamma, const float *beta, float *running_mean, float *running_var,
                       long M, int C, int training, float momentum, float eps, float slope, float *out, float *mean,
                       float *invstd, float *workspace, fsg_stream_t stream);
int fsg_bn_act_bwd_f32(const float *grad_out, const float *y, const float *gamma, const float *beta, const float *mean,
                       const float *invstd, long M, int C, int training, float slope, float *grad_y, float *grad_gamma,
                       float *grad_beta, float *workspace, fsg_stream_t stream);

size_t fsg_bn_act_max_workspace_bytes(int B, int N, int C);
int fsg_bn_act_max_fwd_f32(const float *y, const float *gamma, const float *beta, float *running_mean,
                           float *running_var, int B, int N, int C, int training, float momentum, float eps,
                           float slope, float *out, float *ysel, int32_t *arg, float *mean, float *invstd,
                           float *workspace, fsg_stream_t stream);
int fsg_bn_act_max_bwd_f32(const float *grad_out, const float *y, const float *ysel, const int32_t *arg,
                           const float *gamma, const float *beta, const float *mean, const float *invstd, int B, int N,
                           int C, int training, float slope, float *grad_y, float *grad_gamma, float *grad_beta,
                           fsg_stream_t stream);

size_t fsg_bn_act_maxavg_workspace_bytes(int B, int N, int C);
int fsg_bn_act_maxavg_fwd_f32(const float *y, const float *gamma, const float *beta, float *running_mean,
                              float *running_var, int B, int N, int C, int training, float momentum, float eps,
                              float slope, float *out, int32_t *arg, float *mean, float *invstd, float *workspace,
                              fsg_stream_t stream);
int fsg_bn_act_maxavg_bwd_f32(const float *grad_out, const float *y, const int32_t *arg, const float *gamma,
                              const float *beta, const float *mean, const float *invstd, int B, int N, int C,
                              int training, float slope, float *grad_y, float *grad_gamma, float *grad_beta,
                              float *workspace, fsg_stream_t stream);

size_t fsg_chamfer_nn_bwd_workspace_bytes(int B, int N, int M);
int fsg_chamfer_nn_f32(const float *x, const float *y, int B, int N, int M, float *dist,
                       int32_t *arg, fsg_stream_t stream);
int fsg_chamfer_nn_bwd_f32(const float *x, const float *y, const int32_t *arg, const float *g_dist,
                           int B, int N, int M, float *grad_x, float *grad_y, void *workspace,
                           fsg_stream_t stream);

int fsg_point_mesh_dist_f32(const float *pts, const float *verts, const int32_t *faces, int B, int P, int V, int F,
                            int Bf, float *dist2, int32_t *face, float *closest, fsg_stream_t stream);

int fsg_mesh_labelmap_dist_f32(const float *verts, const int32_t *faces, const int32_t *labels, int V, int F, int d0, int d1,
                               int d2, float s0, float s1, float s2, float dist_threshold, const uint8_t *mask, uint64_t *keys,
                               int64_t *out, fsg_stream_t stream);
int fsg_mesh_labelmap_cover_f32(const float *verts, const int32_t *faces, const int32_t *labels, int V, int F, int d0, int d1,
                                int d2, float s0, float s1, float s2, int64_t *out, fsg_stream_t stream);

size_t fsg_nnu_loss_workspace_bytes(int C);
int fsg_nnu_loss_f32(const float *logits, int64_t stride_b, int64_t stride_c, int64_t stride_n,
                     const int64_t *labels, const float *class_weights, int B, int C, int N, float w_ce,
                     float w_dice, float smooth, float *loss_out, float *grad, int64_t gstride_b,
                     int64_t gstride_c, int64_t gstride_n, void *workspace, fsg_stream_t stream);

int fsg_knn_segment_f32(const float *xyz, const float *new_xyz, const int32_t *offset,
                        const int32_t *new_offset, int b, int n, int m, int nsample, int32_t *idx,
                        float *dist2, fsg_stream_t stream);

int fsg_fps_f32(const float *xyz, const int32_t *offset, const int32_t *new_offset, int b, int n,
                float *tmp, int32_t *idx, fsg_stream_t stream);

int fsg_group_gather_fwd_f32(const float *feat, const int32_t *idx, float *out, int n, int c, int m,
                             int ns, fsg_stream_t stream);
int fsg_group_gather_bwd_f32(const float *grad_out, const int32_t *idx, float *grad_feat, int n,
                             int c, int m, int ns, fsg_stream_t stream);

int fsg_group_xyz_feat_fwd_f32(const float *xyz, const float *new_xyz, const float *feat, const int32_t *idx, float *out, int n,
                               int c, int m, int ns, fsg_stream_t stream);
int fsg_group_xyz_feat_bwd_f32(const float *grad_out, const int32_t *idx, float *grad_feat, int n, int c, int m, int ns,
                               fsg_stream_t stream);

int fsg_rows_max_fwd_f32(const float *x, float *out, int32_t *arg, int m, int ns, int c, fsg_stream_t stream);
int fsg_rows_max_bwd_f32(const float *grad_out, const int32_t *arg, float *grad_x, int m, int ns, int c, fsg_stream_t stream);

int fsg_interp_fwd_f32(const float *feat, const int32_t *idx, const float *dist2, float *out, int n, int c, int m, int k,
                       fsg_stream_t stream);
int fsg_interp_bwd_f32(const float *grad_out, const int32_t *idx, const float *dist2, float *grad_feat, int n, int c, int m, int k,
                       fsg_stream_t stream);


int fsg_vec_attn_fwd_f32(const float *v, const float *pos, const float *w, const int32_t *idx,
                         float *out, int n, int ns, int c, int cw, fsg_stream_t stream);
int fsg_vec_attn_bwd_f32(const float *v, const float *pos, const float *w, const int32_t *idx,
                         const float *grad_out, float *grad_v, float *grad_pos, float *grad_w, int n,
                         int ns, int c, int cw, fsg_stream_t stream);

size_t fsg_bn_rows_workspace_bytes(long M, int C);
int fsg_bn_rows_fwd_f32(const float *x, const float *residual, const float *gamma, const float *beta,
                        float *running_mean, float *running_var, long M, int C, int training, float momentum,
                        float eps, int relu, float *out, float *mean, float *rstd, void *workspace,
                        fsg_stream_t stream);
int fsg_bn_rows_bwd_f32(const float *grad_out, const float *x, const float *out, const float *gamma,
                        const float *mean, const float *rstd, long M, int C, int training, int relu,
                        float *grad_x, float *grad_residual, float *grad_gamma, float *grad_beta,
                        void *workspace, fsg_stream_t stream);

size_t fsg_gemm_small_workspace_bytes(int I, int J, int K);
int fsg_gemm_small_f32(const float *A, int64_t sa_i, int64_t sa_k, const float *B, int64_t sb_k, int64_t sb_j,
                       const float *bias, float *C, int64_t ldc, int I, int J, int K, void *workspace,
                       fsg_stream_t stream);
int fsg_gemm_small_rowsum_f32(const float *A, int64_t sa_i, int64_t sa_k, const float *B, int64_t sb_k, int64_t sb_j,
                              const float *bias, float *C, int64_t ldc, int I, int J, int K, float *rowsum, void *workspace,
                              fsg_stream_t stream);

#define FSG_GEMM_REDUCE_MAX_JOBS 48
typedef struct fsg_gemm_reduce_jobs {
    const float *part[FSG_GEMM_REDUCE_MAX_JOBS];
    float *C[FSG_GEMM_REDUCE_MAX_JOBS];
    float *rowsum[FSG_GEMM_REDUCE_MAX_JOBS];
    int64_t ldc[FSG_GEMM_REDUCE_MAX_JOBS];
    int32_t S[FSG_GEMM_REDUCE_MAX_JOBS], I[FSG_GEMM_REDUCE_MAX_JOBS], J[FSG_GEMM_REDUCE_MAX_JOBS], blocks[FSG_GEMM_REDUCE_MAX_JOBS];
    int32_t n;
} fsg_gemm_reduce_jobs;
int fsg_gemm_small_deferred_f32(const float *A, int64_t sa_i, int64_t sa_k, const float *B, int64_t sb_k, int64_t sb_j, float *C,
                                int64_t ldc, int I, int J, int K, float *rowsum, void *workspace, int *splits,
                                fsg_stream_t stream);
int fsg_gemm_small_reduce_many_f32(const fsg_gemm_reduce_jobs *jobs, fsg_stream_t stream);
int fsg_gemm_small_bf16(const float *A, int64_t sa_i, int64_t sa_k, const float *B, int64_t sb_k, int64_t sb_j, const float *bias,
                        float *C, int64_t ldc, int I, int J, int K, float *rowsum, void *workspace, int *splits,
                        fsg_stream_t stream);


typedef struct fsg_pt_layer_params {
    const float *lp1_w, *lp1_b;
    const float *bnp_g, *bnp_b;
    float *bnp_rm, *bnp_rv;
    const float *lp2_w, *lp2_b;
    const float *bn1_g, *bn1_b;
    float *bn1_rm, *bn1_rv;
    const float *lw1_w, *lw1_b;
    const float *bn2_g, *bn2_b;
    float *bn2_rm, *bn2_rv;
    const float *lw2_w, *lw2_b;
    float eps_p, eps_1, eps_2;
    float mom_p, mom_1, mom_2;
} fsg_pt_layer_params;

typedef struct fsg_pt_layer_grads {
    float *lp1_w, *lp1_b, *bnp_g, *bnp_b, *lp2_w, *lp2_b, *bn1_g, *bn1_b, *lw1_w, *lw1_b, *bn2_g, *bn2_b, *lw2_w,
        *lw2_b;
} fsg_pt_layer_grads;

size_t fsg_pt_attn_workspace_bytes(int n, int ns, int c);
int fsg_pt_attn_fwd_f32(const float *p, const int32_t *idx, const float *q, const float *k, const float *v,
                        int64_t ld, const fsg_pt_layer_params *params, int n, int ns, int c, int training,
                        float *out, float *stats, float *u1, float *sm, void *workspace, fsg_stream_t stream);
int fsg_pt_attn_bwd_f32(const float *p, const int32_t *idx, const float *q, const float *k, const float *v,
                        int64_t ld, const fsg_pt_layer_params *params, int n, int ns, int c, int training,
                        const float *grad_out, const float *stats, const float *u1, const float *sm,
                        float *grad_q, float *grad_k, float *grad_v, int64_t ldg, float *grad_p,
                        const fsg_pt_layer_grads *grads, void *workspace, fsg_stream_t stream);

int fsg_adam_flat_f32(float *param, const float *grad, float *exp_avg, float *exp_avg_sq, void *state, int64_t n,
                      float lr, const float *lr_dev, float beta1, float beta2, float eps, float weight_decay,
                      fsg_stream_t stream);

size_t fsg_ensemble_accumulate_workspace_bytes(int R, int64_t n_points);
int fsg_ensemble_accumulate_f32(const float *logits, int R, int B, int cls, int S, const int64_t *pts, int64_t n_points,
                                float *acc, void *workspace, fsg_stream_t stream);

int fsg_sample_transform_f32(const float *x, int B, int C, int64_t N, const int64_t *sample, int S, const float *affine,
                             float *out, fsg_stream_t stream);

#define FSG_SSM_MAX_MODES 64
size_t fsg_ssm_decode_bwd_workspace_bytes(int B, int P, int M);
int fsg_ssm_decode_fwd_f32(const float *w, const float *mean, const float *evec, const float *v, const float *s,
                           const float *tr, int B, int P, int M, float *out, fsg_stream_t stream);
int fsg_ssm_decode_bwd_f32(const float *grad_out, const float *w, const float *mean, const float *evec, const float *v,
                           const float *s, int B, int P, int M, float *grad_w, float *grad_v, float *grad_s, float *grad_tr,
                           void *workspace, size_t workspace_bytes, fsg_stream_t stream);

int fsg_colsum_narrow_f32(const float *x, int64_t M, int C, float *out, fsg_stream_t stream);

int fsg_fold_layer1_f32(const float *pts, int cp, const float *w, int64_t ldw, const float *per_cloud, int B, int m, int Cout,
                        int relu, float *out, fsg_stream_t stream);

#define FSG_PW_MAX_IMAGE_JOBS 10
typedef struct fsg_pw_image_jobs {
    const float *W[FSG_PW_MAX_IMAGE_JOBS];
    int64_t stride_n[FSG_PW_MAX_IMAGE_JOBS], stride_k[FSG_PW_MAX_IMAGE_JOBS];
    int N[FSG_PW_MAX_IMAGE_JOBS], K[FSG_PW_MAX_IMAGE_JOBS], ks0[FSG_PW_MAX_IMAGE_JOBS], KS[FSG_PW_MAX_IMAGE_JOBS];
    float scale[FSG_PW_MAX_IMAGE_JOBS];
    void *image[FSG_PW_MAX_IMAGE_JOBS];
    int n;
} fsg_pw_image_jobs;
int fsg_pw_weight_images_f32(const fsg_pw_image_jobs *jobs, fsg_stream_t stream);
size_t fsg_pw_weight_image_bytes(int N, int K);
int fsg_pw_weight_image_f32(const float *W, int64_t stride_n, int64_t stride_k, int N, int K, float scale, int ks0, int KS,
                            void *image, fsg_stream_t stream);
int fsg_pw_linear_f32(const float *A, int64_t lda, const void *image, const float *bias, float *C, int64_t ldc, int M, int N,
                      int K, int tile, fsg_stream_t stream);

int fsg_pw_weight_image_bf16(const float *W, int64_t stride_n, int64_t stride_k, int N, int K, void *image, fsg_stream_t stream);
int fsg_pw_linear_bf16(const float *A, int64_t lda, const void *image, const float *bias, float *C, int64_t ldc, int M, int N,
                       int K, int tile, fsg_stream_t stream);

typedef struct fsg_pw_rowgemm_args {
    const float *A1, *Y1, *A2;
    int64_t lda1, lda2;
    int K1, K2;
    const void *Bimg;
    int M, N, rows_per_cloud;
    const float *alpha, *delta, *P, *Q;
    int tstride;
    float slope;
    float *C;
    int64_t ldc;
    int store_n0;
    const float *bias;
    float *rec;
    const float *sgn;
    float *sel_val;
    int32_t *sel_arg;
    int sel_n;
    const float *Yp;
    int64_t ldyp;
    const float *ealpha, *edelta, *emu, *er;
    int etstride;
    float *rec2;
} fsg_pw_rowgemm_args;
int fsg_pw_tile_rows(int tile);
int fsg_pw_rowgemm_f32(const fsg_pw_rowgemm_args *args, int pro, int epi, int tile, fsg_stream_t stream);

typedef struct fsg_pw_tn_args {
    const float *L1, *LY1, *L2;
    int64_t ldl1, ldl2;
    int N1a, N1b, lpro;
    const float *lalpha, *ldelta, *lP, *lQ;
    int lts;
    const float *R;
    int64_t ldr;
    int N2, rpro;
    const float *ralpha, *rdelta;
    int rts;
    float slope;
    int M, rows_per_cloud, rows_per_slice;
    int ones;
} fsg_pw_tn_args;
#define FSG_PW_MAX_REDUCE_JOBS 6
typedef struct fsg_pw_tn_reduce_jobs {
    const void *workspace[FSG_PW_MAX_REDUCE_JOBS];
    float *C1[FSG_PW_MAX_REDUCE_JOBS], *C2[FSG_PW_MAX_REDUCE_JOBS];
    int64_t ldc1[FSG_PW_MAX_REDUCE_JOBS], ldc2[FSG_PW_MAX_REDUCE_JOBS];
    int S[FSG_PW_MAX_REDUCE_JOBS], N1[FSG_PW_MAX_REDUCE_JOBS], N2[FSG_PW_MAX_REDUCE_JOBS], N1a[FSG_PW_MAX_REDUCE_JOBS];
    int n;
} fsg_pw_tn_reduce_jobs;
int fsg_pw_tn_reduce_f32(const fsg_pw_tn_reduce_jobs *jobs, fsg_stream_t stream);
size_t fsg_pw_tn_workspace_bytes(int N1, int N2, int M, int rows_per_slice);
int fsg_pw_tn_f32(const fsg_pw_tn_args *args, int tile, void *workspace, size_t workspace_bytes, float *C1, int64_t ldc1,
                  float *C2, int64_t ldc2, fsg_stream_t stream);
int fsg_pw_tn_bf16(const fsg_pw_tn_args *args, int tile, void *workspace, size_t workspace_bytes, float *C1, int64_t ldc1,
                   fsg_stream_t stream);

int fsg_pw_bn_finalize_f32(const float *rec, int R, int ldn, int c0, int C, const float *shift, int B, int training,
                           const float *gamma, const float *beta, float eps, float momentum, float *running_mean,
                           float *running_var, float *mean, float *invstd, float *alpha, float *delta, float *emu,
                           float *cloud_mean, const float *gfeat, const float *Wglob, int64_t ldwg, int CG, float *shift_out,
                           fsg_stream_t stream);
int fsg_pw_cloud_linear_f32(const float *x, const float *W, int64_t ldw, int B, int C0, int CG, float *out, fsg_stream_t stream);
int fsg_pw_max_finish_f32(const float *sel_val, const int32_t *sel_arg, const float *sgn, const float *alpha, const float *delta,
                          int B, int tiles, int C, float slope, float *out, float *ysel, int32_t *arg, fsg_stream_t stream);
int fsg_pw_bn_finalize_max_f32(const float *rec, int R, int ldn, int c0, int C, int B, int training, const float *gamma,
                               const float *beta, float eps, float momentum, float *running_mean, float *running_var, float *mean,
                               float *invstd, float *alpha, float *delta, const float *sel_val, const int32_t *sel_arg,
                               const float *sgn, int tiles, float slope, float *out, float *ysel, int32_t *arg, fsg_stream_t stream);

int fsg_pw_bnbwd_finalize_f32(const float *rec2, int R, int C, int B, int64_t M, int training, const float *alpha,
                              const float *invstd, const float *emu, int emu_per_cloud, const float *cloud_mean, float *dbeta,
                              float *dgamma, float *P, float *Q, float *dc, fsg_stream_t stream);
int fsg_pw_logits_bwd_f32(const float *g, int classes, const float *W3, const float *y, const float *alpha, const float *delta,
                          const float *mean, const float *invstd, int64_t M, int C, float slope, float *da, float *rec2,
                          fsg_stream_t stream);

int fsg_pw_gf_prep_f32(const float *dc, const float *W0g, int64_t ldw0, int C0, const float *gfeat, float *dW0g, int64_t lddw0,
                       const float *dg, const float *ysel, const float *alpha, const float *delta, const float *mean,
                       const float *invstd, int B, int C, int64_t M, int training, float slope, float *dbeta, float *dgamma,
                       float *P, float *Q, float *coef, const float *W, int64_t ldw, int K, float *Wq, int64_t ldwq,
                       fsg_stream_t stream);
size_t fsg_pw_scatter_rows_workspace_bytes(int B, int C);
int fsg_pw_scatter_rows_f32(const float *coef, const int32_t *arg, const float *W, int64_t ldw, int B, int C, int K, int Npts,
                            float *dX, int64_t ldx, void *workspace, fsg_stream_t stream);
int fsg_pw_gf_dw_f32(const float *coef, const int32_t *arg, const float *X, int64_t ldx, const float *s, const float *W,
                     int64_t ldw, const float *G, const float *P, const float *Q, int B, int C, int K, int Npts, float *dW,
                     int64_t lddw, fsg_stream_t stream);

int fsg_pw_logits_bwd_bias_f32(const float *g, int classes, const float *W3, const float *y, const float *alpha,
                               const float *delta, const float *mean, const float *invstd, int64_t M, int C, float slope,
                               float *da, float *rec2, float *db, fsg_stream_t stream);
int fsg_pw_gf_prep_sort_f32(const float *dc, const float *W0g, int64_t ldw0, int C0, const float *gfeat, float *dW0g, int64_t lddw0,
                            const float *ysel, const float *alpha, const float *delta, const float *mean, const float *invstd,
                            int B, int C, int64_t M, int training, float slope, float *dbeta, float *dgamma, float *P, float *Q,
                            float *coef, const float *W, int64_t ldw, int K, float *Wq, int64_t ldwq, const int32_t *arg, int Npts,
                            void *sorted, int32_t *first, fsg_stream_t stream);
int fsg_pw_tn_reduce_image_f32(const void *workspace, int S, int N1, int N2, int NI, float scale, int ks0, int KS, void *image,
                               float *C2, int64_t ldc2, fsg_stream_t stream);
int fsg_pw_rowgemm_scatter_f32(const fsg_pw_rowgemm_args *args, const void *sorted, const int32_t *first, const float *coef,
                               const float *W, int64_t ldw, int C, fsg_stream_t stream);

int fsg_foerstner_dist_f32(const float *img, int B, int D, int H, int W, const float *weights, int N, float *out,
                           fsg_stream_t stream);
int fsg_nms_keypoints(const float *dist, const uint8_t *mask, int B, int D, int H, int W, int d, float thresh, float *maxout,
                      uint8_t *flags, fsg_stream_t stream);
size_t fsg_mind_stats_workspace_bytes(int B, int D, int H, int W);
int fsg_mind_stats_f32(const float *img, int B, int D, int H, int W, int dilation, int nch, int box, const int *shifts,
                       const float *weights, int N, void *workspace, float *mean, fsg_stream_t stream);
int fsg_mind_eval_f32(const float *img, int B, int D, int H, int W, int dilation, int nch, int box, const int *shifts,
                      const int *outch, const float *weights, int N, const float *mean, float *out, fsg_stream_t stream);
int fsg_mind_eval_kp_f32(const float *img, int D, int H, int W, int dilation, int nch, int box, const int *shifts,
                         const int *outch, const float *weights, int N, const float *mean, const int64_t *kp, int K, float *out,
                         fsg_stream_t stream);

int fsg_fissure_enhance_f32(const float *img, const uint8_t *mask, int B, int D, int H, int W, const float *k1, const float *k2,
                            int N, float mu, float sigma_hu, float *out, float *planeness, float *hu_weight,
                            fsg_stream_t stream);
int fsg_smooth_threshold_f32(const float *vol, int B, int D, int H, int W, const float *wz, int Nz, const float *wy, int Ny,
                             const float *wx, int Nx, float thresh, float *out, uint8_t *flags, fsg_stream_t stream);

size_t fsg_cpd_estep_workspace_bytes(int B, int N, int M);
int fsg_cpd_estep_f32(const float *X, int64_t x_batch_stride, const float *TY, const float *sigma2, float w, int B, int N, int M,
                      float *P1, float *Pt1, float *PX, float *Np, void *workspace, size_t workspace_bytes,
                      fsg_stream_t stream);

#define FSG_RW_BINARY 0
#define FSG_RW_INTENSITY 1
size_t fsg_random_walk_workspace_bytes(int B, int K, int D, int H, int W);
int fsg_random_walk_prep(const void *im, int mode, const void *labels, int labels_are_i32, const uint8_t *mask, int B, int K, int D,
                         int H, int W, void *workspace, size_t workspace_bytes, int32_t *stop_iter, float *relres,
                         fsg_stream_t stream);
int fsg_random_walk_iterate(const void *im, int mode, int B, int K, int D, int H, int W, int first_iteration, int iterations,
                            float tol, void *workspace, size_t workspace_bytes, int32_t *stop_iter, float *relres,
                            fsg_stream_t stream);
int fsg_random_walk_finish(int B, int K, int D, int H, int W, const void *workspace, size_t workspace_bytes, float *prob,
                           uint8_t *filled, fsg_stream_t stream);
int fsg_lobes_to_fissures_u8(const uint8_t *lobes, int B, int D, int H, int W, int n_lobes, uint8_t *fissures,
                             fsg_stream_t stream);

int fsg_bits_pack_u8(const uint8_t *vol, int B, int D, int H, int W, int value, uint64_t *bits, fsg_stream_t stream);
int fsg_bits_unpack_u8(const uint64_t *bits, int B, int D, int H, int W, uint8_t *vol, fsg_stream_t stream);
int fsg_bits_window(const uint64_t *in, int B, int Di, int Hi, int Wi, int oz, int oy, int ox, int Do, int Ho, int Wo,
                    uint64_t *out, fsg_stream_t stream);
int fsg_ball_dilate_bits(const uint64_t *in, int B, int D, int H, int W, int rz, int ry, int rx, int border, int inv_in,
                         int inv_out, uint64_t *out, fsg_stream_t stream);
size_t fsg_cc_workspace_bytes(int B, int D, int H, int W);
int fsg_cc_label_bits(const uint64_t *bits, int B, int D, int H, int W, int connectivity, int32_t *labels, int32_t *n,
                      void *workspace, size_t workspace_bytes, fsg_stream_t stream);
int fsg_component_stats_i32(const int32_t *labels, int B, int D, int H, int W, int cap, int64_t *stats, fsg_stream_t stream);
int fsg_relabel_lut_i32(const int32_t *labels, int B, int64_t n_per_item, const int32_t *lut, int lut_len, void *out,
                        int out_is_i64, fsg_stream_t stream);

size_t fsg_mesh_reg_workspace_bytes(int N, int max_V);
int fsg_mesh_reg_f32(const float *verts, int64_t total_verts, const int32_t *desc, int N, int max_V, const int32_t *nbr_off,
                     const int32_t *nbr, const int32_t *pairs, const int32_t *inc_off, const int32_t *inc, float *terms,
                     float *mean, float *grads, void *workspace, size_t workspace_bytes, fsg_stream_t stream);
size_t fsg_mesh_sample_workspace_bytes(int N, int max_F);
int fsg_mesh_sample_f32(const float *verts, const int32_t *faces, const int32_t *sdesc, int N, int max_F, const float *u, int n,
                        float *pts, int32_t *face, float *w, void *workspace, size_t workspace_bytes, fsg_stream_t stream);
int fsg_mesh_sample_bwd_f32(const float *g, const int32_t *face, const float *w, const int32_t *faces, const int32_t *sdesc,
                            int N, int max_V, int n, float *grad_verts, fsg_stream_t stream);

#define FSG_GRID_TORCH 0
#define FSG_GRID_SAP 1
int fsg_grid_corners_f32(const float *coords, int B, int N, int D, int H, int W, int mode, int32_t *keys, float *w,
                         fsg_stream_t stream);
size_t fsg_grid_splat_workspace_bytes(int B, int C, int N);
int fsg_grid_splat_sorted_f32(const float *values, const int32_t *keys_sorted, const int64_t *perm, const float *w, int B, int C,
                              int N, int D, int H, int W, float *grid, void *workspace, size_t workspace_bytes,
                              fsg_stream_t stream);
int fsg_grid_sample_f32(const float *grid, const float *coords, const float *weights, int B, int C, int N, int D, int H, int W,
                        int mode, float *sampled, float *grad_coords, fsg_stream_t stream);
int fsg_psr_spectral_f32(const float *in, int B, int R0, int R1, int R2, double sig, int adjoint, float *out,
                         fsg_stream_t stream);

size_t fsg_mc_workspace_bytes(int B, int D, int H, int W);
int fsg_mc_count_f32(const float *field, const uint8_t *mask, int64_t mask_item_stride, int B, int D, int H, int W, float isolevel,
                     int validate, void *workspace, size_t workspace_bytes, int64_t *totals, fsg_stream_t stream);
int fsg_mc_count_labels_i32(const int32_t *labels, const uint8_t *mask, int64_t mask_item_stride, int first_label, int B, int D,
                            int H, int W, void *workspace, size_t workspace_bytes, int64_t *totals, fsg_stream_t stream);
int fsg_mc_emit_f32(const float *field, int B, int D, int H, int W, float isolevel, int local_coords, float sx, float sy, float sz,
                    const void *workspace, size_t workspace_bytes, const int64_t *totals, int64_t total_verts, int64_t total_faces,
                    float *verts, int64_t *faces, float *normals, fsg_stream_t stream);
int fsg_mc_emit_labels_i32(const int32_t *labels, int first_label, int B, int D, int H, int W, int local_coords, float sx, float sy,
                           float sz, const void *workspace, size_t workspace_bytes, const int64_t *totals, int64_t total_verts,
                           int64_t total_faces, float *verts, int64_t *faces, float *normals, fsg_stream_t stream);

int fsg_pcl_normals_f32(const float *xyz, const int32_t *idx, const int32_t *offset, int b, int n, int K, int disambiguate,
                        float *normals, float *curvatures, float *frames, fsg_stream_t stream);

size_t fsg_orient_normals_workspace_bytes(int n, int K);
int fsg_orient_normals_f32(const float *xyz, const float *normals, const int32_t *idx, const int32_t *offset, int b, int n, int K,
                           void *workspace, size_t workspace_bytes, float *out, int8_t *signs, int32_t *comp, fsg_stream_t stream);
int fsg_face_union_i32(const int64_t *sorted_keys, const int64_t *half_edge, int F, int32_t *parent, int32_t *root,
                       fsg_stream_t stream);
int fsg_cluster_stats_f64(const float *verts, const int32_t *faces, const int32_t *sorted_clusters, const int64_t *face_order,
                          const int64_t *sorted_vertex_keys, int V, int F, int C, double *area, int64_t *num_verts, double *vert_sum,
                          fsg_stream_t stream);
int fsg_mesh_keep_flags_u8(const float *verts, int V, const int32_t *vert_offset, int B, const uint8_t *keep_in, const float *boxes,
                           const uint8_t *mask, int D, int H, int W, float sx, float sy, float sz, uint8_t *keep, fsg_stream_t stream);
int fsg_mesh_face_flags_u8(const int32_t *faces, int V, int F, const uint8_t *vert_keep, const uint8_t *face_keep, uint8_t *face_out,
                           uint8_t *vert_used, fsg_stream_t stream);
int fsg_mesh_compact_f32(const float *verts, const float *normals, const int32_t *faces, int V, int F, const int32_t *vert_offset,
                         int B, const uint8_t *vert_flag, const int64_t *vert_new, const uint8_t *face_flag, const int64_t *face_new,
                         float *verts_out, float *normals_out, int64_t *faces_out, fsg_stream_t stream);

#ifdef __cplusplus
}
#endif
#endif
```

Measured before the change: 17.37 million.

## Fuse grad gather into segmented Adam and batch deferred weight-grad GEMMs

Adds a segmented Adam kernel that reads per-parameter gradients directly, writes them into the flat gradient buffer and applies the update in one launch, replacing a separate gather step. The edge-weight backward now launches all pending weight-gradient GEMMs as one batched deferred job and folds their split-K reduction into the edge-weight backward kernel. It also software-pipelines the loads in the flat Adam kernel. Together these cut kernel launches and intermediate copies during backward and the optimizer step, at the cost of more complex bookkeeping across autograd slots and fallback paths.

```diff
diff --git a/fissure-segmentation_amd/_lib.py b/fissure-segmentation_amd/_lib.py
--- a/fissure-segmentation_amd/_lib.py
+++ b/fissure-segmentation_amd/_lib.py
@@ -34,6 +34,7 @@
     "fsg_edge_weights_fwd_f32": ([_P, _I, _I, _P, _P], _I),
     "fsg_edge_weights_bwd_f32": ([_P, _I, _I, _P, _P], _I),
     "fsg_edge_weights_many_f32": ([_P, _I, _P], _I),
+    "fsg_edge_weights_bwd_folded_f32": ([_P, _P], _I),
     "fsg_edgeconv1_workspace_bytes": ([_I, _I, _I], ctypes.c_size_t),
     "fsg_edgeconv1_fwd_f32": ([_P, _P, _P, _P, _P, _P, _I, _I, _I, _I, _I, _F, _F, _F, _P, _P, _P, _P, _P, _P, _P, _P, _P],
                               _I),
@@ -69,6 +70,7 @@
     "fsg_colsum_narrow_f32": ([_P, _L, _I, _P, _P], _I),
     "fsg_fold_layer1_f32": ([_P, _I, _P, _L, _P, _I, _I, _I, _I, _P, _P], _I),
     "fsg_adam_flat_f32": ([_P, _P, _P, _P, _P, _L, _F, _P, _F, _F, _F, _F, _P], _I),
+    "fsg_adam_flat_segments_f32": ([_P, _P, _P, _P, _P, _L, _P, _F, _P, _F, _F, _F, _F, _P], _I),
     "fsg_nnu_loss_workspace_bytes": ([_I], ctypes.c_size_t),
     "fsg_nnu_loss_f32": ([_P, _L, _L, _L, _P, _P, _I, _I, _I, _F, _F, _F, _P, _P, _L, _L, _L, _P, _P], _I),
     "fsg_bn_rows_workspace_bytes": ([ctypes.c_long, _I], ctypes.c_size_t),
@@ -79,6 +81,7 @@
     "fsg_gemm_small_rowsum_f32": ([_P, _L, _L, _P, _L, _L, _P, _P, _L, _I, _I, _I, _P, _P, _P], _I),
     "fsg_gemm_small_deferred_f32": ([_P, _L, _L, _P, _L, _L, _P, _L, _I, _I, _I, _P, _P, _P, _P], _I),
     "fsg_gemm_small_reduce_many_f32": ([_P, _P], _I),
+    "fsg_gemm_small_many_deferred_f32": ([_P, _P], _I),
     "fsg_gemm_small_bf16": ([_P, _L, _L, _P, _L, _L, _P, _P, _L, _I, _I, _I, _P, _P, _P, _P], _I),
     "fsg_pt_attn_workspace_bytes": ([_I, _I, _I], ctypes.c_size_t),
     "fsg_pt_attn_fwd_f32": ([_P, _P, _P, _P, _P, _L, _P, _I, _I, _I, _I, _P, _P, _P, _P, _P, _P], _I),
@@ -215,8 +218,26 @@
                 ("J", _I * GEMM_REDUCE_MAX_JOBS), ("blocks", _I * GEMM_REDUCE_MAX_JOBS), ("n", _I)]
 
 
+ADAM_MAX_SEGMENTS = 128
+
+
+class AdamSegments(ctypes.Structure):
+    _fields_ = [("grad", _P * ADAM_MAX_SEGMENTS), ("offset", _L * ADAM_MAX_SEGMENTS), ("count", _L * ADAM_MAX_SEGMENTS),
+                ("n", _I)]
+
+
+class GemmSmallJobs(ctypes.Structure):
+    _fields_ = [("A", _P * 8), ("sa_i", _L * 8), ("sa_k", _L * 8), ("B", _P * 8), ("sb_k", _L * 8), ("sb_j", _L * 8),
+                ("C", _P * 8), ("ldc", _L * 8), ("I", _I * 8), ("J", _I * 8), ("K", _I * 8), ("workspace", _P * 8),
+                ("splits", _I * 8), ("n", _I)]
+
+
 class EdgeWeightJobs(ctypes.Structure):
     _fields_ = [("src", _P * 8), ("dst", _P * 8), ("Co", _I * 8), ("C", _I * 8), ("n", _I)]
+
+
+class EdgeWeightFoldJobs(ctypes.Structure):
+    _fields_ = [("src", _P * 8), ("dst", _P * 8), ("Co", _I * 8), ("C", _I * 8), ("S", _I * 8), ("n", _I)]
 
 
 class PWRowGemmArgs(ctypes.Structure):
diff --git a/fissure-segmentation_amd/csrc/adam.hip b/fissure-segmentation_amd/csrc/adam.hip
--- a/fissure-segmentation_amd/csrc/adam.hip
+++ b/fissure-segmentation_amd/csrc/adam.hip
@@ -1,6 +1,8 @@
 #include "fsg_common.h"
 
 namespace {
+
+constexpr int FSG_ADAM_MAX_CHUNKS = 224;
 
 struct AdamState {
     float step;
@@ -16,12 +18,8 @@
     p -= step_size * (m / denom);
 }
 
-__global__ __launch_bounds__(256) void adam_flat_kernel(float *__restrict__ param, const float *__restrict__ grad,
-                                                        float *__restrict__ exp_avg, float *__restrict__ exp_avg_sq,
-                                                        AdamState *__restrict__ state, long n, float lr_host,
-                                                        const float *__restrict__ lr_dev, float b1, float b2, float eps,
-                                                        float wd) {
-    __shared__ float sc[2];
+__device__ __forceinline__ void adam_bias_terms(float *sc, const AdamState *state, float lr_host, const float *lr_dev, float b1,
+                                                float b2) {
     if (threadIdx.x == 0) {
         const double t = (double)state->step + 1.0;
         const double lr = lr_dev ? (double)lr_dev[0] : (double)lr_host;
@@ -29,37 +27,107 @@
         sc[1] = (float)sqrt(1.0 - pow((double)b2, t));
     }
     __syncthreads();
-    const float step_size = sc[0], bc2_sqrt = sc[1];
-    const long n4 = n >> 2;
-    for (long i = (long)blockIdx.x * 256 + threadIdx.x; i < n4; i += (long)gridDim.x * 256) {
-        float4 p = reinterpret_cast<float4 *>(param)[i];
-        const float4 g = reinterpret_cast<const float4 *>(grad)[i];
-        float4 m = reinterpret_cast<float4 *>(exp_avg)[i];
-        float4 v = reinterpret_cast<float4 *>(exp_avg_sq)[i];
-        adam_one(p.x, g.x, m.x, v.x, b1, b2, eps, wd, step_size, bc2_sqrt);
-        adam_one(p.y, g.y, m.y, v.y, b1, b2, eps, wd, step_size, bc2_sqrt);
-        adam_one(p.z, g.z, m.z, v.z, b1, b2, eps, wd, step_size, bc2_sqrt);
-        adam_one(p.w, g.w, m.w, v.w, b1, b2, eps, wd, step_size, bc2_sqrt);
-        reinterpret_cast<float4 *>(param)[i] = p;
-        reinterpret_cast<float4 *>(exp_avg)[i] = m;
-        reinterpret_cast<float4 *>(exp_avg_sq)[i] = v;
-    }
-    if (blockIdx.x == 0 && threadIdx.x < (n & 3)) {
-        const long i = (n4 << 2) + threadIdx.x;
-        float p = param[i], m = exp_avg[i], v = exp_avg_sq[i];
-        adam_one(p, grad[i], m, v, b1, b2, eps, wd, step_size, bc2_sqrt);
-        param[i] = p;
-        exp_avg[i] = m;
-        exp_avg_sq[i] = v;
-    }
+}
+
+__device__ __forceinline__ void adam_four(float4 &p, const float4 &g, float4 &m, float4 &v, float b1, float b2, float eps, float wd,
+                                          float step_size, float bc2_sqrt) {
+    adam_one(p.x, g.x, m.x, v.x, b1, b2, eps, wd, step_size, bc2_sqrt);
+    adam_one(p.y, g.y, m.y, v.y, b1, b2, eps, wd, step_size, bc2_sqrt);
+    adam_one(p.z, g.z, m.z, v.z, b1, b2, eps, wd, step_size, bc2_sqrt);
+    adam_one(p.w, g.w, m.w, v.w, b1, b2, eps, wd, step_size, bc2_sqrt);
+}
+
+__device__ __forceinline__ void adam_finish(AdamState *state, unsigned int workgroups) {
     __syncthreads();
     if (threadIdx.x == 0) {
         const unsigned int done = atomicAdd(&state->ticket, 1u);
-        if (done == gridDim.x - 1) {
+        if (done == workgroups - 1) {
             state->step += 1.f;
             state->ticket = 0u;
         }
     }
+}
+
+__global__ __launch_bounds__(256) void adam_flat_kernel(float *__restrict__ param, const float *__restrict__ grad,
+                                                        float *__restrict__ exp_avg, float *__restrict__ exp_avg_sq,
+                                                        AdamState *__restrict__ state, long n, float lr_host,
+                                                        const float *__restrict__ lr_dev, float b1, float b2, float eps,
+                                                        float wd) {
+    __shared__ float sc[2];
+    const long n4 = n >> 2, stride = (long)gridDim.x * 256;
+    long i = (long)blockIdx.x * 256 + threadIdx.x;
+    float4 p, g, m, v;
+    if (i < n4) {
+        p = reinterpret_cast<float4 *>(param)[i];
+        g = reinterpret_cast<const float4 *>(grad)[i];
+        m = reinterpret_cast<float4 *>(exp_avg)[i];
+        v = reinterpret_cast<float4 *>(exp_avg_sq)[i];
+    }
+    adam_bias_terms(sc, state, lr_host, lr_dev, b1, b2);
+    const float step_size = sc[0], bc2_sqrt = sc[1];
+    while (i < n4) {
+        adam_four(p, g, m, v, b1, b2, eps, wd, step_size, bc2_sqrt);
+        reinterpret_cast<float4 *>(param)[i] = p;
+        reinterpret_cast<float4 *>(exp_avg)[i] = m;
+        reinterpret_cast<float4 *>(exp_avg_sq)[i] = v;
+        i += stride;
+        if (i < n4) {
+            p = reinterpret_cast<float4 *>(param)[i];
+            g = reinterpret_cast<const float4 *>(grad)[i];
+            m = reinterpret_cast<float4 *>(exp_avg)[i];
+            v = reinterpret_cast<float4 *>(exp_avg_sq)[i];
+        }
+    }
+    if (blockIdx.x == 0 && threadIdx.x < (n & 3)) {
+        const long t = (n4 << 2) + threadIdx.x;
+        float pt = param[t], mt = exp_avg[t], vt = exp_avg_sq[t];
+        adam_one(pt, grad[t], mt, vt, b1, b2, eps, wd, step_size, bc2_sqrt);
+        param[t] = pt;
+        exp_avg[t] = mt;
+        exp_avg_sq[t] = vt;
+    }
+    adam_finish(state, gridDim.x);
+}
+
+struct AdamChunks {
+    const float *grad[FSG_ADAM_MAX_CHUNKS];
+    unsigned int off[FSG_ADAM_MAX_CHUNKS], count[FSG_ADAM_MAX_CHUNKS];
+};
+
+__global__ __launch_bounds__(1024) void adam_flat_segments_kernel(float *__restrict__ param, float *flat_grad,
+                                                                 float *__restrict__ exp_avg, float *__restrict__ exp_avg_sq,
+                                                                 AdamState *__restrict__ state, AdamChunks chunks, float lr_host,
+                                                                 const float *__restrict__ lr_dev, float b1, float b2, float eps,
+                                                                 float wd) {
+    __shared__ float sc[2];
+    const float4 *src = reinterpret_cast<const float4 *>(chunks.grad[blockIdx.x]);
+    const long base = chunks.off[blockIdx.x];
+    const unsigned int cnt = chunks.count[blockIdx.x], stride = 1024;
+    unsigned int i = threadIdx.x;
+    float4 p, g, m, v;
+    if (i < cnt) {
+        p = reinterpret_cast<float4 *>(param)[base + i];
+        g = src[i];
+        m = reinterpret_cast<float4 *>(exp_avg)[base + i];
+        v = reinterpret_cast<float4 *>(exp_avg_sq)[base + i];
+    }
+    adam_bias_terms(sc, state, lr_host, lr_dev, b1, b2);
+    const float step_size = sc[0], bc2_sqrt = sc[1];
+    while (i < cnt) {
+        reinterpret_cast<float4 *>(flat_grad)[base + i] = g;
+        adam_four(p, g, m, v, b1, b2, eps, wd, step_size, bc2_sqrt);
+        reinterpret_cast<float4 *>(param)[base + i] = p;
+        reinterpret_cast<float4 *>(exp_avg)[base + i] = m;
+        reinterpret_cast<float4 *>(exp_avg_sq)[base + i] = v;
+        i += stride;
+        if (i < cnt) {
+            p = reinterpret_cast<float4 *>(param)[base + i];
+            g = src[i];
+            m = reinterpret_cast<float4 *>(exp_avg)[base + i];
+            v = reinterpret_cast<float4 *>(exp_avg_sq)[base + i];
+        }
+    }
+    adam_finish(state, gridDim.x);
 }
 
 }
@@ -82,3 +150,42 @@
     FSG_CHECK_LAUNCH("fsg_adam_flat_f32");
     return FSG_OK;
 }
+
+extern "C" int fsg_adam_flat_segments_f32(float *param, float *flat_grad, float *exp_avg, float *exp_avg_sq, void *state, int64_t n,
+                                          const fsg_adam_segments *segments, float lr, const float *lr_dev, float beta1,
+                                          float beta2, float eps, float weight_decay, fsg_stream_t stream) {
+    FSG_REQUIRE(param && flat_grad && exp_avg && exp_avg_sq && state && segments, "fsg_adam_flat_segments_f32: NULL pointer");
+    FSG_REQUIRE(n > 0 && n < (1L << 33), "fsg_adam_flat_segments_f32: n=%ld", (long)n);
+    FSG_REQUIRE((((uintptr_t)param | (uintptr_t)flat_grad | (uintptr_t)exp_avg | (uintptr_t)exp_avg_sq) & 15) == 0,
+                "fsg_adam_flat_segments_f32: the four arrays must be 16-byte aligned");
+    FSG_REQUIRE(((uintptr_t)state & 7) == 0, "fsg_adam_flat_segments_f32: state must be 8-byte aligned");
+    FSG_REQUIRE(beta1 >= 0.f && beta1 < 1.f && beta2 >= 0.f && beta2 < 1.f && eps >= 0.f,
+                "fsg_adam_flat_segments_f32: bad hyper-parameters beta1=%g beta2=%g eps=%g", beta1, beta2, eps);
+    const int ns = segments->n;
+    FSG_REQUIRE(ns >= 1 && ns <= FSG_ADAM_MAX_SEGMENTS, "fsg_adam_flat_segments_f32: 1..%d segments", FSG_ADAM_MAX_SEGMENTS);
+    int64_t at = 0;
+    for (int s = 0; s < ns; ++s) {
+        FSG_REQUIRE(segments->grad[s] && ((uintptr_t)segments->grad[s] & 15) == 0 && segments->count[s] > 0 &&
+                        (segments->count[s] & 3) == 0 && segments->offset[s] == at,
+                    "fsg_adam_flat_segments_f32: segment %d must be 16-byte aligned, a multiple of 4 floats and start where "
+                    "segment %d ends", s, s - 1);
+        at += segments->count[s];
+    }
+    FSG_REQUIRE(at == n, "fsg_adam_flat_segments_f32: the segments cover %ld of %ld elements", (long)at, (long)n);
+    const long n4 = n >> 2, per = fsg_cdiv(n4, (long)(FSG_ADAM_MAX_CHUNKS - ns));
+    AdamChunks ch;
+    int nc = 0;
+    for (int s = 0; s < ns; ++s) {
+        const long c4 = segments->count[s] >> 2, o4 = segments->offset[s] >> 2;
+        for (long c0 = 0; c0 < c4; c0 += per, ++nc) {
+            ch.grad[nc] = segments->grad[s] + 4 * c0;
+            ch.off[nc] = (unsigned int)(o4 + c0);
+            ch.count[nc] = (unsigned int)(c4 - c0 < per ? c4 - c0 : per);
+        }
+    }
+    for (int c = nc; c < FSG_ADAM_MAX_CHUNKS; ++c) ch.grad[c] = nullptr, ch.off[c] = ch.count[c] = 0;
+    hipLaunchKernelGGL(adam_flat_segments_kernel, dim3((unsigned)nc), dim3(1024), 0, (hipStream_t)stream, param,
+                       flat_grad, exp_avg, exp_avg_sq, (AdamState *)state, ch, lr, lr_dev, beta1, beta2, eps, weight_decay);
+    FSG_CHECK_LAUNCH("fsg_adam_flat_segments_f32");
+    return FSG_OK;
+}
diff --git a/fissure-segmentation_amd/csrc/small_gemm.hip b/fissure-segmentation_amd/csrc/small_gemm.hip
--- a/fissure-segmentation_amd/csrc/small_gemm.hip
+++ b/fissure-segmentation_amd/csrc/small_gemm.hip
@@ -5,6 +5,76 @@
 
 constexpr int TI = 64, TJ = 64, TK = 32, LDT = 65;
 constexpr int LPT = TI * TK / 256;
+
+__device__ __forceinline__ void gemm_small_tile(const float *__restrict__ A, long sai, long sak, const float *__restrict__ B,
+                                                long sbk, long sbj, const float *__restrict__ bias, float *__restrict__ C, long ldc,
+                                                int I, int J, int K, int kchunk, float *__restrict__ part,
+                                                float *__restrict__ rowsum, int bx, int by, int bz, int nz, float *As, float *Bs) {
+    const int tid = threadIdx.x, wave = __builtin_amdgcn_readfirstlane(tid >> 6), lane = tid & 63, ql = lane & 31, half = lane >> 5;
+    const int i0 = bx * TI, j0 = by * TJ;
+    const int kbeg = bz * kchunk, kend = min(K, kbeg + kchunk);
+    const int wi = (wave >> 1) * 32, wj = (wave & 1) * 32;
+    const bool a_kfast = sak == 1, b_kfast = sbk == 1;
+    f32x16 acc;
+#pragma unroll
+    for (int e = 0; e < 16; ++e) acc[e] = 0.f;
+    float av[LPT], bv[LPT];
+    auto fetch = [&](int k0) {
+#pragma unroll
+        for (int r = 0; r < LPT; ++r) {
+            const int t = r * 256 + tid;
+            const int ai = a_kfast ? t / TK : t % TI, ak = a_kfast ? t % TK : t / TI;
+            const int bj = b_kfast ? t / TK : t % TJ, bk = b_kfast ? t % TK : t / TJ;
+            av[r] = (i0 + ai < I && k0 + ak < kend) ? A[(long)(i0 + ai) * sai + (long)(k0 + ak) * sak] : 0.f;
+            bv[r] = (j0 + bj < J && k0 + bk < kend) ? B[(long)(k0 + bk) * sbk + (long)(j0 + bj) * sbj] : 0.f;
+        }
+    };
+    const bool do_rs = rowsum != nullptr && by == 0 && tid < TI;
+    float rs = 0.f;
+    if (kbeg < kend) fetch(kbeg);
+    for (int k0 = kbeg; k0 < kend; k0 += TK) {
+        __syncthreads();
+#pragma unroll
+        for (int r = 0; r < LPT; ++r) {
+            const int t = r * 256 + tid;
+            const int ai = a_kfast ? t / TK : t % TI, ak = a_kfast ? t % TK : t / TI;
+            const int bj = b_kfast ? t / TK : t % TJ, bk = b_kfast ? t % TK : t / TJ;
+            As[ak * LDT + ai] = av[r];
+            Bs[bk * LDT + bj] = bv[r];
+        }
+        __syncthreads();
+        if (k0 + TK < kend) fetch(k0 + TK);
+        if (do_rs) {
+#pragma unroll
+            for (int kk = 0; kk < TK; ++kk) rs += As[kk * LDT + tid];
+        }
+#pragma unroll
+        for (int s = 0; s < TK / 2; ++s)
+            acc = __builtin_amdgcn_mfma_f32_32x32x2f32(As[(2 * s + half) * LDT + wi + ql], Bs[(2 * s + half) * LDT + wj + ql],
+                                                       acc, 0, 0, 0);
+    }
+    if (do_rs && i0 + tid < I) {
+        if (part) part[(long)nz * I * J + (long)bz * I + i0 + tid] = rs;
+        else rowsum[i0 + tid] = rs;
+    }
+    const int col = j0 + wj + ql;
+    if (col >= J) return;
+    if (part) {
+        float *dst = part + (long)bz * I * J;
+#pragma unroll
+        for (int e = 0; e < 16; ++e) {
+            const int row = i0 + wi + (e & 3) + 8 * (e >> 2) + 4 * half;
+            if (row < I) dst[(long)row * J + col] = acc[e];
+        }
+    } else {
+        const float bb = bias ? bias[col] : 0.f;
+#pragma unroll
+        for (int e = 0; e < 16; ++e) {
+            const int row = i0 + wi + (e & 3) + 8 * (e >> 2) + 4 * half;
+            if (row < I) C[(long)row * ldc + col] = acc[e] + bb;
+        }
+    }
+}
 
 __global__ __launch_bounds__(256) void gemm_small_kernel(const float *__restrict__ A, long sai, long sak,
                                                          const float *__restrict__ B, long sbk, long sbj,
@@ -12,70 +82,30 @@
                                                          int I, int J, int K, int kchunk, float *__restrict__ part,
                                                          float *__restrict__ rowsum) {
     __shared__ float As[TK * LDT], Bs[TK * LDT];
-    const int tid = threadIdx.x, wave = __builtin_amdgcn_readfirstlane(tid >> 6), lane = tid & 63, ql = lane & 31, half = lane >> 5;
-    const int i0 = blockIdx.x * TI, j0 = blockIdx.y * TJ;
-    const int kbeg = blockIdx.z * kchunk, kend = min(K, kbeg + kchunk);
-    const int wi = (wave >> 1) * 32, wj = (wave & 1) * 32;
-    const bool a_kfast = sak == 1, b_kfast = sbk == 1;
-    f32x16 acc;
-#pragma unroll
-    for (int e = 0; e < 16; ++e) acc[e] = 0.f;
-    float av[LPT], bv[LPT];
-    auto fetch = [&](int k0) {
-#pragma unroll
-        for (int r = 0; r < LPT; ++r) {
-            const int t = r * 256 + tid;
-            const int ai = a_kfast ? t / TK : t % TI, ak = a_kfast ? t % TK : t / TI;
-            const int bj = b_kfast ? t / TK : t % TJ, bk = b_kfast ? t % TK : t / TJ;
-            av[r] = (i0 + ai < I && k0 + ak < kend) ? A[(long)(i0 + ai) * sai + (long)(k0 + ak) * sak] : 0.f;
-            bv[r] = (j0 + bj < J && k0 + bk < kend) ? B[(long)(k0 + bk) * sbk + (long)(j0 + bj) * sbj] : 0.f;
-        }
-    };
-    const bool do_rs = rowsum != nullptr && blockIdx.y == 0 && tid < TI;
-    float rs = 0.f;
-    if (kbeg < kend) fetch(kbeg);
-    for (int k0 = kbeg; k0 < kend; k0 += TK) {
-        __syncthreads();
-#pragma unroll
-        for (int r = 0; r < LPT; ++r) {
-            const int t = r * 256 + tid;
-            const int ai = a_kfast ? t / TK : t % TI, ak = a_kfast ? t % TK : t / TI;
-            const int bj = b_kfast ? t / TK : t % TJ, bk = b_kfast ? t % TK : t / TJ;
-            As[ak * LDT + ai] = av[r];
-            Bs[bk * LDT + bj] = bv[r];
-        }
-        __syncthreads();
-        if (k0 + TK < kend) fetch(k0 + TK);
-        if (do_rs) {
-#pragma unroll
-            for (int kk = 0; kk < TK; ++kk) rs += As[kk * LDT + tid];
-        }
-#pragma unroll
-        for (int s = 0; s < TK / 2; ++s)
-            acc = __builtin_amdgcn_mfma_f32_32x32x2f32(As[(2 * s + half) * LDT + wi + ql], Bs[(2 * s + half) * LDT + wj + ql],
-                                                       acc, 0, 0, 0);
-    }
-    if (do_rs && i0 + tid < I) {
-        if (part) part[(long)gridDim.z * I * J + (long)blockIdx.z * I + i0 + tid] = rs;
-        else rowsum[i0 + tid] = rs;
-    }
-    const int col = j0 + wj + ql;
-    if (col >= J) return;
-    if (part) {
-        float *dst = part + (long)blockIdx.z * I * J;
-#pragma unroll
-        for (int e = 0; e < 16; ++e) {
-            const int row = i0 + wi + (e & 3) + 8 * (e >> 2) + 4 * half;
-            if (row < I) dst[(long)row * J + col] = acc[e];
-        }
-    } else {
-        const float bb = bias ? bias[col] : 0.f;
-#pragma unroll
-        for (int e = 0; e < 16; ++e) {
-            const int row = i0 + wi + (e & 3) + 8 * (e >> 2) + 4 * half;
-            if (row < I) C[(long)row * ldc + col] = acc[e] + bb;
-        }
-    }
+    gemm_small_tile(A, sai, sak, B, sbk, sbj, bias, C, ldc, I, J, K, kchunk, part, rowsum, blockIdx.x, blockIdx.y, blockIdx.z,
+                    gridDim.z, As, Bs);
+}
+
+struct SmallGemmJobs {
+    const float *A[FSG_GEMM_SMALL_MAX_JOBS], *B[FSG_GEMM_SMALL_MAX_JOBS];
+    float *C[FSG_GEMM_SMALL_MAX_JOBS], *part[FSG_GEMM_SMALL_MAX_JOBS];
+    long sai[FSG_GEMM_SMALL_MAX_JOBS], sak[FSG_GEMM_SMALL_MAX_JOBS], sbk[FSG_GEMM_SMALL_MAX_JOBS], sbj[FSG_GEMM_SMALL_MAX_JOBS];
+    long ldc[FSG_GEMM_SMALL_MAX_JOBS];
+    int I[FSG_GEMM_SMALL_MAX_JOBS], J[FSG_GEMM_SMALL_MAX_JOBS], K[FSG_GEMM_SMALL_MAX_JOBS], kchunk[FSG_GEMM_SMALL_MAX_JOBS];
+    int ti[FSG_GEMM_SMALL_MAX_JOBS], tj[FSG_GEMM_SMALL_MAX_JOBS], S[FSG_GEMM_SMALL_MAX_JOBS];
+    int first[FSG_GEMM_SMALL_MAX_JOBS];
+    int n;
+};
+__global__ __launch_bounds__(256) void gemm_small_many_kernel(SmallGemmJobs jobs) {
+    __shared__ float As[TK * LDT], Bs[TK * LDT];
+    int j = 0;
+    while (j + 1 < jobs.n && (int)blockIdx.x >= jobs.first[j + 1]) ++j;
+    int b = blockIdx.x - jobs.first[j];
+    const int bx = b % jobs.ti[j];
+    b /= jobs.ti[j];
+    const int by = b % jobs.tj[j], bz = b / jobs.tj[j];
+    gemm_small_tile(jobs.A[j], jobs.sai[j], jobs.sak[j], jobs.B[j], jobs.sbk[j], jobs.sbj[j], nullptr, jobs.C[j], jobs.ldc[j],
+                    jobs.I[j], jobs.J[j], jobs.K[j], jobs.kchunk[j], jobs.part[j], nullptr, bx, by, bz, jobs.S[j], As, Bs);
 }
 
 typedef unsigned short u16;
@@ -212,6 +242,67 @@
     }
 }
 
+constexpr int SLICED_MIN_S = 16;
+
+constexpr int FOLD_BATCH = 8;
+__device__ __forceinline__ void fold_sum2(const float *__restrict__ part, long IJ, long ip, long iq, int s_begin, int s_step, int S,
+                                          float &ap, float &aq) {
+    for (int s0 = s_begin; s0 < S; s0 += s_step * FOLD_BATCH) {
+        float vp[FOLD_BATCH], vq[FOLD_BATCH];
+#pragma unroll
+        for (int u = 0; u < FOLD_BATCH; ++u) {
+            const int s = s0 + s_step * u;
+            vp[u] = s < S ? part[(long)s * IJ + ip] : 0.f;
+            vq[u] = s < S ? part[(long)s * IJ + iq] : 0.f;
+        }
+#pragma unroll
+        for (int u = 0; u < FOLD_BATCH; ++u)
+            if (s0 + s_step * u < S) {
+                ap += vp[u];
+                aq += vq[u];
+            }
+    }
+}
+__global__ __launch_bounds__(256) void edge_weights_bwd_folded_kernel(fsg_edge_weight_fold_jobs jobs) {
+    __shared__ float red[2][16][17];
+    const int j = blockIdx.y;
+    const int Co = jobs.Co[j], C = jobs.C[j], S = jobs.S[j];
+    const int o = threadIdx.x & 15, sl = threadIdx.x >> 4;
+    const int t = blockIdx.x * 16 + o;
+    const bool live = t < Co * C;
+    const float *__restrict__ src = jobs.src[j];
+    const long IJ = 2L * Co * C;
+    const int r = t / C, c = t - r * C;
+    const long ip = (long)r * C + c, iq = (long)(Co + r) * C + c;
+    float gp = 0.f, gq = 0.f;
+    if (S >= SLICED_MIN_S) {
+        float ap = 0.f, aq = 0.f;
+        if (live) fold_sum2(src, IJ, ip, iq, sl, 16, S, ap, aq);
+        red[0][sl][o] = ap;
+        red[1][sl][o] = aq;
+        __syncthreads();
+        if (sl == 0) {
+#pragma unroll
+            for (int i = 0; i < 16; ++i) {
+                gp += red[0][i][o];
+                gq += red[1][i][o];
+            }
+        }
+    } else if (sl == 0 && live) {
+        if (S > 1) {
+            fold_sum2(src, IJ, ip, iq, 0, 1, S, gp, gq);
+        } else {
+            gp = src[ip];
+            gq = src[iq];
+        }
+    }
+    if (sl == 0 && live) {
+        float *dst = jobs.dst[j] + (long)r * 2 * C;
+        dst[c] = gp - gq;
+        dst[C + c] = gq;
+    }
+}
+
 __global__ __launch_bounds__(256) void gemm_small_reduce_many_kernel(fsg_gemm_reduce_jobs jobs) {
     int j = 0;
     long b = blockIdx.x;
@@ -302,6 +393,50 @@
     FSG_REQUIRE(total < (1L << 31), "fsg_gemm_small_reduce_many_f32: too many outputs");
     hipLaunchKernelGGL(gemm_small_reduce_many_kernel, dim3((unsigned)total), dim3(256), 0, (hipStream_t)stream, j);
     FSG_CHECK_LAUNCH("fsg_gemm_small_reduce_many_f32");
+    return FSG_OK;
+}
+
+extern "C" int fsg_gemm_small_many_deferred_f32(fsg_gemm_small_jobs *jobs, fsg_stream_t stream) {
+    FSG_REQUIRE(jobs && jobs->n >= 1 && jobs->n <= FSG_GEMM_SMALL_MAX_JOBS, "fsg_gemm_small_many_deferred_f32: 1..%d jobs",
+                FSG_GEMM_SMALL_MAX_JOBS);
+    SmallGemmJobs t = {};
+    t.n = jobs->n;
+    long total = 0;
+    for (int j = 0; j < jobs->n; ++j) {
+        const int I = jobs->I[j], J = jobs->J[j], K = jobs->K[j];
+        FSG_REQUIRE(jobs->A[j] && jobs->B[j] && jobs->C[j], "fsg_gemm_small_many_deferred_f32: NULL pointer in job %d", j);
+        FSG_REQUIRE(I > 0 && J > 0 && K > 0 && jobs->ldc[j] >= J, "fsg_gemm_small_many_deferred_f32: bad shape I=%d J=%d K=%d in job %d",
+                    I, J, K, j);
+        const int S = splits_for(I, J, K);
+        FSG_REQUIRE(S == 1 || jobs->workspace[j], "fsg_gemm_small_many_deferred_f32: job %d needs the workspace", j);
+        const int kchunk = fsg_cdiv(fsg_cdiv(K, S), TK) * TK, S_eff = fsg_cdiv(K, kchunk);
+        t.A[j] = jobs->A[j], t.B[j] = jobs->B[j], t.C[j] = jobs->C[j];
+        t.part[j] = S_eff > 1 ? (float *)jobs->workspace[j] : nullptr;
+        t.sai[j] = jobs->sa_i[j], t.sak[j] = jobs->sa_k[j], t.sbk[j] = jobs->sb_k[j], t.sbj[j] = jobs->sb_j[j], t.ldc[j] = jobs->ldc[j];
+        t.I[j] = I, t.J[j] = J, t.K[j] = K, t.kchunk[j] = kchunk, t.ti[j] = fsg_cdiv(I, TI), t.tj[j] = fsg_cdiv(J, TJ), t.S[j] = S_eff;
+        t.first[j] = (int)total;
+        total += (long)t.ti[j] * t.tj[j] * S_eff;
+        FSG_REQUIRE(total < (1L << 31), "fsg_gemm_small_many_deferred_f32: too many workgroups");
+        jobs->splits[j] = S_eff > 1 ? S_eff : 0;
+    }
+    hipLaunchKernelGGL(gemm_small_many_kernel, dim3((unsigned)total), dim3(256), 0, (hipStream_t)stream, t);
+    FSG_CHECK_LAUNCH("fsg_gemm_small_many_deferred_f32");
+    return FSG_OK;
+}
+
+extern "C" int fsg_edge_weights_bwd_folded_f32(const fsg_edge_weight_fold_jobs *jobs, fsg_stream_t stream) {
+    FSG_REQUIRE(jobs && jobs->n >= 1 && jobs->n <= FSG_EDGE_WEIGHT_MAX_JOBS, "fsg_edge_weights_bwd_folded_f32: 1..%d jobs",
+                FSG_EDGE_WEIGHT_MAX_JOBS);
+    long most = 0;
+    for (int j = 0; j < jobs->n; ++j) {
+        FSG_REQUIRE(jobs->src[j] && jobs->dst[j] && jobs->Co[j] > 0 && jobs->C[j] > 0 && jobs->S[j] >= 0 &&
+                        2L * jobs->Co[j] * jobs->C[j] < (1L << 31),
+                    "fsg_edge_weights_bwd_folded_f32: bad job %d", j);
+        const long e = (long)jobs->Co[j] * jobs->C[j];
+        most = e > most ? e : most;
+    }
+    hipLaunchKernelGGL(edge_weights_bwd_folded_kernel, dim3(fsg_cdiv(most, 16), jobs->n), dim3(256), 0, (hipStream_t)stream, *jobs);
+    FSG_CHECK_LAUNCH("fsg_edge_weights_bwd_folded_f32");
     return FSG_OK;
 }
 
@@ -331,7 +466,7 @@
     }
     if (part) {
         const long IJ = (long)I * J, outs = IJ + (rowsum ? I : 0);
-        if (S_eff >= 16)
+        if (S_eff >= SLICED_MIN_S)
             hipLaunchKernelGGL(gemm_small_reduce_kernel, dim3(fsg_cdiv(IJ, 16) + (rowsum ? fsg_cdiv(I, 16) : 0)), dim3(256), 0, st, part,
                                S_eff, IJ, J, bias, C, (long)ldc, I, rowsum);
         else
diff --git a/fissure-segmentation_amd/functional.py b/fissure-segmentation_amd/functional.py
--- a/fissure-segmentation_amd/functional.py
+++ b/fissure-segmentation_amd/functional.py
@@ -270,6 +270,7 @@
         ctx.save_for_backward(x, w)
         ctx.has_bias = b is not None
         ctx.pw16 = False
+        ctx.fold = _fold_slot(w)
         tw, tb = _grad_targets(w), (_grad_targets(b) if b is not None else ())
         ctx.defer_targets = tw + tb if (tw is not None and tb is not None) else None
         x2 = x.reshape(-1, x.shape[-1])
@@ -299,6 +300,8 @@
         gx = gw = gb = None
         if not g2.is_contiguous():
             g2 = g2.contiguous()
+        if ctx.fold is not None:
+            ctx.fold.pending = None
         if ctx.gs16:
             N, K = w.shape
             M = g2.shape[0]
@@ -324,7 +327,9 @@
         if ctx.needs_input_grad[0]:
             gx = _linear_dx(g2, w).view_as(x)
         want_gb = ctx.has_bias and ctx.needs_input_grad[2]
-        if ctx.needs_input_grad[1]:
+        if ctx.needs_input_grad[1] and not want_gb and x2.is_contiguous():
+            gw = _dw_unreduced(ctx.fold, w, g2, x2)
+        if ctx.needs_input_grad[1] and gw is None:
             gw = _linear_dw(g2, x2, with_bias_grad=want_gb, defer=_may_defer(ctx.defer_targets))
             if isinstance(gw, tuple):
                 gw, gb = gw
@@ -352,6 +357,43 @@
     return g2.t() @ x2
 
 
+_fused_pq_tail = True
+
+
+def set_fused_pq_tail(flag):
+    global _fused_pq_tail
+    old, _fused_pq_tail = _fused_pq_tail, bool(flag)
+    return old
+
+
+class _FoldSlot:
+    __slots__ = ("uses", "pending")
+
+    def __init__(self):
+        self.uses, self.pending = 0, None
+
+
+def _fold_slot(w):
+    slot = getattr(w, "_fsg_fold", None)
+    if slot is not None:
+        slot.uses += 1
+    return slot
+
+
+def _dw_unreduced(slot, w, g2, x2):
+    if slot is None:
+        return None
+    slot.pending = None
+    M, N = g2.shape
+    K = x2.shape[1]
+    if not _fused_pq_tail or slot.uses != 1 or torch.is_grad_enabled() or w.retains_grad or w._backward_hooks or \
+            not _small(N, K, M, g2, x2):
+        return None
+    out = torch.empty(N, K, dtype=torch.float32, device=g2.device)
+    slot.pending = (out, g2, x2)
+    return out
+
+
 def _bias_grad(g2):
     M, N = g2.shape
     if g2.is_cuda and g2.dtype == torch.float32 and N <= 32 and (N & (N - 1)) == 0 and 4096 <= M * N <= 131072:
@@ -368,6 +410,7 @@
     @_amp_fwd
     def forward(ctx, x, w, value):
         ctx.save_for_backward(x, w)
+        ctx.fold = _fold_slot(w)
         return value.view_as(value)
 
     @staticmethod
@@ -379,7 +422,12 @@
             g2 = g2.contiguous()
         x2 = x.reshape(-1, x.shape[-1])
         gx = _linear_dx(g2, w).view_as(x) if ctx.needs_input_grad[0] else None
-        gw = _linear_dw(g2, x2 if x2.is_contiguous() else x2.contiguous()) if ctx.needs_input_grad[1] else None
+        gw = None
+        if ctx.needs_input_grad[1]:
+            x2 = x2 if x2.is_contiguous() else x2.contiguous()
+            gw = _dw_unreduced(ctx.fold, w, g2, x2)
+            if gw is None:
+                gw = _linear_dw(g2, x2)
         return gx, gw, None
 
 
@@ -579,9 +627,10 @@
 
     @staticmethod
     @_amp_fwd
-    def forward(ctx, *Ws):
+    def forward(ctx, slots, *Ws):
         Wc = [W if (W.dtype == torch.float32 and W.is_contiguous()) else W.float().contiguous() for W in Ws]
         ctx.shapes = [(W.shape[0], W.shape[1] // 2) for W in Wc]
+        ctx.slots = slots
         return tuple(_EdgeWeightsMany._run(Wc, ctx.shapes, False))
 
     @staticmethod
@@ -591,14 +640,52 @@
         gc = [torch.zeros(2 * Co, C, dtype=torch.float32, device=dev) if g is None else
               (g if (g.dtype == torch.float32 and g.is_contiguous()) else g.float().contiguous())
               for g, (Co, C) in zip(gs, ctx.shapes)]
-        return tuple(_EdgeWeightsMany._run(gc, ctx.shapes, True))
+        pending = [None] * len(gc)
+        for j, slot in enumerate(ctx.slots or ()):
+            pending[j], slot.pending = slot.pending, None
+        if not any(pending):
+            return (None,) + tuple(_EdgeWeightsMany._run(gc, ctx.shapes, True))
+        prods = _lib.GemmSmallJobs()
+        spaces = []
+        for j, pend in enumerate(pending):
+            if pend is None:
+                continue
+            dw, g2, x2 = pend
+            if gs[j] is None or gs[j].data_ptr() != dw.data_ptr():
+                raise RuntimeError("edge_weights_many: the gradient of weight %d is not the product that was registered for it "
+                                   "(a weight of edge_weights_many may feed one product only)" % j)
+            (M, N), K, i = g2.shape, x2.shape[1], len(spaces)
+            ws = _lib.workspace("fsg_gemm_small", N, K, M, device=dev)
+            prods.A[i], prods.sa_i[i], prods.sa_k[i], prods.B[i], prods.sb_k[i], prods.sb_j[i] = g2.data_ptr(), 1, N, x2.data_ptr(), K, 1
+            prods.C[i], prods.ldc[i], prods.I[i], prods.J[i], prods.K[i] = dw.data_ptr(), K, N, K, M
+            prods.workspace[i] = ws.data_ptr() if ws is not None else None
+            spaces.append((j, ws))
+        prods.n = len(spaces)
+        jobs = _lib.EdgeWeightFoldJobs()
+        jobs.n = len(gc)
+        outs = []
+        with torch.cuda.device(dev):
+            _lib.call("fsg_gemm_small_many_deferred_f32", ctypes.byref(prods), _stream())
+            partials = {j: (ws, prods.splits[i]) for i, (j, ws) in enumerate(spaces)}
+            for j, (g, (Co, C)) in enumerate(zip(gc, ctx.shapes)):
+                ws, S = partials.get(j, (None, 0))
+                out = torch.empty(Co, 2 * C, dtype=torch.float32, device=dev)
+                jobs.src[j], jobs.dst[j] = (ws if S > 1 else g).data_ptr(), out.data_ptr()
+                jobs.Co[j], jobs.C[j], jobs.S[j] = Co, C, S
+                outs.append(out)
+            _lib.call("fsg_edge_weights_bwd_folded_f32", ctypes.byref(jobs), _stream())
+        return (None,) + tuple(outs)
 
 
 def edge_weights_many(conv_weights):
     Ws = [w.reshape(w.shape[0], w.shape[1]) for w in conv_weights]
     if not 1 <= len(Ws) <= 8:
         raise ValueError("edge_weights_many: 1..8 layers")
-    return list(_EdgeWeightsMany.apply(*Ws))
+    slots = [_FoldSlot() for _ in Ws]
+    outs = list(_EdgeWeightsMany.apply(slots, *Ws))
+    for w, slot in zip(outs, slots):
+        w._fsg_fold = slot
+    return outs
 
 
 _deferred_counters = None
diff --git a/fissure-segmentation_amd/optim.py b/fissure-segmentation_amd/optim.py
--- a/fissure-segmentation_amd/optim.py
+++ b/fissure-segmentation_amd/optim.py
@@ -58,6 +58,9 @@
         if self.inner is not None:
             self.inner.step()
             return
+        self._launch("fsg_adam_flat_f32", None)
+
+    def _launch(self, entry, segments):
         from . import _lib
         g = self._groups[0]
         lr = g["lr"]
@@ -67,11 +70,35 @@
                 raise ValueError("a tensor learning rate must be one fp32 element on the parameters' device")
             lr_dev, lr = ctypes.c_void_p(lr.data_ptr()), 0.0
         P = lambda t: ctypes.c_void_p(t.data_ptr())
-        _lib.call("fsg_adam_flat_f32", P(self.flat.data), P(self.flat.grad), P(self.exp_avg), P(self.exp_avg_sq),
-                  P(self._state), self.flat.numel(), float(lr), lr_dev, float(g["betas"][0]), float(g["betas"][1]),
-                  float(g["eps"]), float(g["weight_decay"]), ctypes.c_void_p(torch.cuda.current_stream().cuda_stream))
+        table = () if segments is None else (segments,)
+        with torch.cuda.device(self.flat.device):
+            _lib.call(entry, P(self.flat.data), P(self.flat.grad), P(self.exp_avg), P(self.exp_avg_sq),
+                      P(self._state), self.flat.numel(), *table, float(lr), lr_dev, float(g["betas"][0]), float(g["betas"][1]),
+                      float(g["eps"]), float(g["weight_decay"]), ctypes.c_void_p(torch.cuda.current_stream().cuda_stream))
+
+    def _grad_segments(self):
+        from . import _lib
+        if self.inner is not None or len(self.params) > _lib.ADAM_MAX_SEGMENTS:
+            return None
+        seg = _lib.AdamSegments()
+        for i, (p, (a, b)) in enumerate(zip(self.params, self._spans)):
+            g = p.grad
+            if g is None or g.dtype != torch.float32 or g.device != self.flat.device or not g.is_contiguous() or \
+                    g.numel() != b - a or (a | b) & 3 or g.data_ptr() & 15:
+                return None
+            seg.grad[i], seg.offset[i], seg.count[i] = g.data_ptr(), a, b - a
+        seg.n = len(self.params)
+        return seg
 
     def step(self):
+        seg = None
+        if self.inner is None:
+            from . import functional as F_hip
+            F_hip.flush_deferred_reduces()
+            seg = self._grad_segments()
+        if seg is not None:
+            self._launch("fsg_adam_flat_segments_f32", ctypes.byref(seg))
+            return
         missing = [i for i, p in enumerate(self.params) if p.grad is None]
         self.gather_grads()
         if not missing or self.inner is not None:
diff --git a/include/fsg_hip.h b/include/fsg_hip.h
--- a/include/fsg_hip.h
+++ b/include/fsg_hip.h
@@ -71,6 +71,15 @@
     int n;
 } fsg_edge_weight_jobs;
 int fsg_edge_weights_many_f32(const fsg_edge_weight_jobs *jobs, int backward, fsg_stream_t stream);
+typedef struct fsg_edge_weight_fold_jobs {
+    const float *src[FSG_EDGE_WEIGHT_MAX_JOBS];
+    float *dst[FSG_EDGE_WEIGHT_MAX_JOBS];
+    int Co[FSG_EDGE_WEIGHT_MAX_JOBS];
+    int C[FSG_EDGE_WEIGHT_MAX_JOBS];
+    int S[FSG_EDGE_WEIGHT_MAX_JOBS];
+    int n;
+} fsg_edge_weight_fold_jobs;
+int fsg_edge_weights_bwd_folded_f32(const fsg_edge_weight_fold_jobs *jobs, fsg_stream_t stream);
 
 int fsg_edgeconv_apply_f32(const float *ysel, const float *gamma, const float *beta, const float *mean, const float *invstd,
                            int B, int N, int Co, float slope, float *out, float *out_pm, void *knn_workspace,
@@ -240,6 +249,20 @@
                                 int64_t ldc, int I, int J, int K, float *rowsum, void *workspace, int *splits,
                                 fsg_stream_t stream);
 int fsg_gemm_small_reduce_many_f32(const fsg_gemm_reduce_jobs *jobs, fsg_stream_t stream);
+#define FSG_GEMM_SMALL_MAX_JOBS 8
+typedef struct fsg_gemm_small_jobs {
+    const float *A[FSG_GEMM_SMALL_MAX_JOBS];
+    int64_t sa_i[FSG_GEMM_SMALL_MAX_JOBS], sa_k[FSG_GEMM_SMALL_MAX_JOBS];
+    const float *B[FSG_GEMM_SMALL_MAX_JOBS];
+    int64_t sb_k[FSG_GEMM_SMALL_MAX_JOBS], sb_j[FSG_GEMM_SMALL_MAX_JOBS];
+    float *C[FSG_GEMM_SMALL_MAX_JOBS];
+    int64_t ldc[FSG_GEMM_SMALL_MAX_JOBS];
+    int32_t I[FSG_GEMM_SMALL_MAX_JOBS], J[FSG_GEMM_SMALL_MAX_JOBS], K[FSG_GEMM_SMALL_MAX_JOBS];
+    void *workspace[FSG_GEMM_SMALL_MAX_JOBS];
+    int32_t splits[FSG_GEMM_SMALL_MAX_JOBS];
+    int32_t n;
+} fsg_gemm_small_jobs;
+int fsg_gemm_small_many_deferred_f32(fsg_gemm_small_jobs *jobs, fsg_stream_t stream);
 int fsg_gemm_small_bf16(const float *A, int64_t sa_i, int64_t sa_k, const float *B, int64_t sb_k, int64_t sb_j, const float *bias,
                         float *C, int64_t ldc, int I, int J, int K, float *rowsum, void *workspace, int *splits,
                         fsg_stream_t stream);
@@ -278,6 +301,15 @@
 int fsg_adam_flat_f32(float *param, const float *grad, float *exp_avg, float *exp_avg_sq, void *state, int64_t n,
                       float lr, const float *lr_dev, float beta1, float beta2, float eps, float weight_decay,
                       fsg_stream_t stream);
+#define FSG_ADAM_MAX_SEGMENTS 128
+typedef struct fsg_adam_segments {
+    const float *grad[FSG_ADAM_MAX_SEGMENTS];
+    int64_t offset[FSG_ADAM_MAX_SEGMENTS], count[FSG_ADAM_MAX_SEGMENTS];
+    int32_t n;
+} fsg_adam_segments;
+int fsg_adam_flat_segments_f32(float *param, float *flat_grad, float *exp_avg, float *exp_avg_sq, void *state, int64_t n,
+                               const fsg_adam_segments *segments, float lr, const float *lr_dev, float beta1, float beta2,
+                               float eps, float weight_decay, fsg_stream_t stream);
 
 size_t fsg_ensemble_accumulate_workspace_bytes(int R, int64_t n_points);
 int fsg_ensemble_accumulate_f32(const float *logits, int R, int B, int cls, int S, const int64_t *pts, int64_t n_points,
```

Measured after the change: 17.98 million (median of 6 runs). +3.5%, better.
